# YJxyzxyz/road-vision-system

Hardware: AMD Instinct MI355X
Metric: end-to-end frames/sec @1080p (preproc+YOLOv8n+SORT), 1/2/4/8 MI355X (higher is better)
Workload: dtype bf16

## Files before the change

road-vision-system_amd/csrc/conv.hip:

```cpp
#include <algorithm>
#include <cstdlib>
#include <cstring>
#include "conv.h"
#include "conv_common.h"

namespace rv {

template <int MR, int NR, int WC>
__global__ __launch_bounds__(256, 2) void conv_mfma_kernel(ConvArgs a) {
  constexpr int WP = 4 / WC;
  const int tid = threadIdx.x;
  const int wave = tid >> 6, lane = tid & 63;
  const int col = lane & 15, quad = lane >> 4;
  const int wp = wave % WP, wc = wave / WP;
  const int cout_pad = (a.Cout + 15) & ~15;
  const int cout0 = (blockIdx.y * WC + wc) * (16 * MR);
  const int HWo = a.Ho * a.Wo;
  const int M = a.B * HWo;
  const int pix0 = (blockIdx.x * WP + wp) * (16 * NR);
  if (cout0 >= cout_pad || pix0 >= M) return;

  const int cin_pad = (a.Cin + 31) & ~31;
  const int kspt = cin_pad >> 5;
  const int Kp = a.k * a.k * cin_pad;
  const int nks = a.k * kspt;
  const int total = a.k * nks;

  const bf16_t* wrow[MR];
#pragma unroll
  for (int m = 0; m < MR; ++m) {
    int r = cout0 + m * 16 + col;
    r = r < cout_pad ? r : cout_pad - 1;
    wrow[m] = a.w + (size_t)r * Kp + quad * 8;
  }
  int iy0[NR], ix0[NR], pb[NR];
  bool pv[NR];
#pragma unroll
  for (int n = 0; n < NR; ++n) {
    const int p = pix0 + n * 16 + col;
    pv[n] = p < M;
    const int pp = pv[n] ? p : 0;
    const int b = pp / HWo;
    const int r = pp - b * HWo;
    const int oy = r / a.Wo;
    const int ox = r - oy * a.Wo;
    iy0[n] = oy * a.stride - a.pad;
    ix0[n] = ox * a.stride - a.pad;
    pb[n] = b * a.Hin * a.Win * a.in_cs + a.in_co + quad * 8;
  }

  f32x4 acc[MR][NR];
#pragma unroll
  for (int m = 0; m < MR; ++m)
#pragma unroll
    for (int n = 0; n < NR; ++n) acc[m][n] = f32x4{0.f, 0.f, 0.f, 0.f};

  const uint4 zero4 = make_uint4(0, 0, 0, 0);
  auto load = [&](int s, bf16x8 (&A)[MR], bf16x8 (&Bf)[NR]) {
    const int ky = s / nks;
    const int r = s - ky * nks;
    const int kx = r / kspt;
    const int cs = r - kx * kspt;
    const int kcol = s * 32;
#pragma unroll
    for (int m = 0; m < MR; ++m) A[m] = __builtin_bit_cast(bf16x8, *(const uint4*)(wrow[m] + kcol));
    const bool cvalid = cs * 32 + quad * 8 < a.Cin;
#pragma unroll
    for (int n = 0; n < NR; ++n) {
      const int iy = iy0[n] + ky, ix = ix0[n] + kx;
      const bool ok = pv[n] && cvalid && (unsigned)iy < (unsigned)a.Hin &&
                      (unsigned)ix < (unsigned)a.Win;
      uint4 v = zero4;
      if (ok)
        v = *(const uint4*)(a.in + (size_t)pb[n] + ((size_t)iy * a.Win + ix) * a.in_cs + cs * 32);
      Bf[n] = __builtin_bit_cast(bf16x8, v);
    }
  };
  auto mma = [&](const bf16x8 (&A)[MR], const bf16x8 (&Bf)[NR]) {
#pragma unroll
    for (int m = 0; m < MR; ++m)
#pragma unroll
      for (int n = 0; n < NR; ++n)
        acc[m][n] = __builtin_amdgcn_mfma_f32_16x16x32_bf16(A[m], Bf[n], acc[m][n], 0, 0, 0);
  };
  bf16x8 A0[MR], B0[NR], A1[MR], B1[NR];
  load(0, A0, B0);
  for (int s = 0; s < total; s += 2) {
    if (s + 1 < total) load(s + 1, A1, B1);
    mma(A0, B0);
    if (s + 1 >= total) break;
    if (s + 2 < total) load(s + 2, A0, B0);
    mma(A1, B1);
  }

#pragma unroll
  for (int n = 0; n < NR; ++n) {
    if (!pv[n]) continue;
    const int p = pix0 + n * 16 + col;
    const int b = p / HWo;
    const int r = p - b * HWo;
    const int oy = r / a.Wo;
    const int ox = r - oy * a.Wo;
    const size_t opix = (size_t)p;
#pragma unroll
    for (int m = 0; m < MR; ++m) {
      const int co = cout0 + m * 16 + quad * 4;
      if (co >= a.Cout) continue;
      float v[4];
      const float4 bb = *(const float4*)(a.bias + co);
      v[0] = acc[m][n][0] + bb.x;
      v[1] = acc[m][n][1] + bb.y;
      v[2] = acc[m][n][2] + bb.z;
      v[3] = acc[m][n][3] + bb.w;
      if (a.act) {
        silu4(v);
      }
      if (a.res) {
        const uint2 rr = *(const uint2*)(a.res + opix * a.res_cs + a.res_co + co);
        v[0] += bf2f(rr.x & 0xFFFF);
        v[1] += bf2f(rr.x >> 16);
        v[2] += bf2f(rr.y & 0xFFFF);
        v[3] += bf2f(rr.y >> 16);
      }
#pragma unroll
      for (int d = 0; d < 2; ++d) {
        void* outp = d == 0 ? a.out0 : a.out1;
        if (!outp) continue;
        const int cs_ = d == 0 ? a.out0_cs : a.out1_cs;
        const int co_ = (d == 0 ? a.out0_co : a.out1_co) + co;
        const int up = d == 0 ? a.out0_up : a.out1_up;
        if (a.out_f32) {
          float* o = (float*)outp;
          const float4 pk = make_float4(v[0], v[1], v[2], v[3]);
          if (!up) {
            *(float4*)(o + opix * cs_ + co_) = pk;
          } else {
            for (int dy = 0; dy < 2; ++dy)
              for (int dx = 0; dx < 2; ++dx) {
                const size_t q = ((size_t)(b * 2 * a.Ho + 2 * oy + dy) * (2 * a.Wo) + 2 * ox + dx);
                *(float4*)(o + q * cs_ + co_) = pk;
              }
          }
        } else {
          uint16_t* o = (uint16_t*)outp;
          const uint2 pk = make_uint2(pack_bf16x2(v[0], v[1]), pack_bf16x2(v[2], v[3]));
          if (!up) {
            *(uint2*)(o + opix * cs_ + co_) = pk;
          } else {
            for (int dy = 0; dy < 2; ++dy)
              for (int dx = 0; dx < 2; ++dx) {
                const size_t q = ((size_t)(b * 2 * a.Ho + 2 * oy + dy) * (2 * a.Wo) + 2 * ox + dx);
                *(uint2*)(o + q * cs_ + co_) = pk;
              }
          }
        }
      }
    }
  }
}

template <int MR, int NR, int WC>
static void launch_t(const ConvArgs& a, hipStream_t s) {
  constexpr int WP = 4 / WC;
  const int M = a.B * a.Ho * a.Wo;
  const int T = (a.Cout + 15) / 16;
  dim3 grid(ceil_div(M, 16 * NR * WP), ceil_div(T, MR * WC));
  conv_mfma_kernel<MR, NR, WC><<<grid, 256, 0, s>>>(a);
}

static int try_launch_patch(const ConvArgs& a, hipStream_t s, int* st);

static bool vcat(const ConvArgs& a) { return a.split > 0 || a.in_up; }

int launch_conv(const ConvArgs& a, hipStream_t s) {
  int st = 0;
  if (vcat(a)) {
    const int T = (a.Cout + 15) / 16;
    ConvCfg c{1, 1, 1, 1, 1, 1};
    for (const int mr : {8, 4, 2})
      if (T % mr == 0 && conv_cfg_ok(a, ConvCfg{mr, 1, 1, 1, 1, 1})) {
        c.mr = mr;
        break;
      }
    if (!conv_cfg_ok(a, c)) {
      set_error("virtual concat input (split %d, up %d) needs a bf16 1x1 conv", a.split, a.in_up);
      return RV_EINVAL;
    }
    return launch_conv_cfg(a, c, s);
  }
  if (try_launch_patch(a, s, &st)) return st;
  if (a.ch_w) {
    set_error("chained 1x1 conv (Cout %d, k%d s%d) has no patch-kernel configuration", a.Cout, a.k,
              a.stride);
    return RV_EINVAL;
  }
  if (a.in8) {
    set_error("fp8 conv (Cin %d, Cout %d, k%d s%d) has no patch-kernel configuration", a.Cin,
              a.Cout, a.k, a.stride);
    return RV_EINVAL;
  }
  if (a.g2_cout0 > 0) {
    set_error("grouped conv (Cout %d, split %d) has no patch-kernel configuration", a.Cout,
              a.g2_cout0);
    return RV_EINVAL;
  }
  const int T = (a.Cout + 15) / 16;
  const long M = (long)a.B * a.Ho * a.Wo;
  struct Cand {
    int mr, nr;
  };
  static const Cand cands[] = {{4, 4}, {2, 8}, {4, 2}, {2, 4}, {1, 8}, {4, 1}, {2, 2},
                               {1, 4}, {2, 1}, {1, 2}, {1, 1}};
  int MR = 1, NR = 1;
  for (const Cand& c : cands) {
    if (c.mr > T) continue;
    const int waste = ceil_div(T, c.mr) * c.mr - T;
    if (waste > 1 && c.mr > 1) continue;
    const long waves = (long)ceil_div((int)((M + 16 * c.nr - 1) / (16 * c.nr)), 1) * ceil_div(T, c.mr);
    MR = c.mr;
    NR = c.nr;
    if (waves >= 2048) break;
  }
  const int groups_c = ceil_div(T, MR);
  const int WC = groups_c >= 4 ? 4 : (groups_c >= 2 ? 2 : 1);
#define RV_CONV_WC(mr, nr)                                           \
  if (MR == mr && NR == nr) {                                        \
    if (WC == 4) launch_t<mr, nr, 4>(a, s);                          \
    else if (WC == 2) launch_t<mr, nr, 2>(a, s);                     \
    else launch_t<mr, nr, 1>(a, s);                                  \
    return launch_status("conv_mfma");                               \
  }
  RV_CONV_WC(4, 4) RV_CONV_WC(2, 8) RV_CONV_WC(4, 2) RV_CONV_WC(2, 4) RV_CONV_WC(1, 8)
  RV_CONV_WC(4, 1) RV_CONV_WC(2, 2) RV_CONV_WC(1, 4) RV_CONV_WC(2, 1) RV_CONV_WC(1, 2)
  RV_CONV_WC(1, 1)
#undef RV_CONV_WC
  set_error("no conv variant for MR=%d NR=%d", MR, NR);
  return RV_EINVAL;
}

__device__ __attribute__((aligned(64))) uint4 g_zero16[4];
#ifdef RV_PHASE_PROF
__device__ unsigned long long g_conv_phase[8];
#define RV_PH_T() __builtin_amdgcn_s_memtime()
#endif

struct TileWalk {
  int t0, step, end;
  __device__ __forceinline__ int count() const { return t0 < end ? (end - t0 + step - 1) / step : 0; }
};
__device__ __forceinline__ TileWalk tile_walk(int ntiles) {
  const int gx = gridDim.x, bx = blockIdx.x;
  if ((gx & 7) == 0) {
    const int chunk = (ntiles + 7) >> 3, j = bx & 7;
    return TileWalk{j * chunk + (bx >> 3), gx >> 3, min(ntiles, (j + 1) * chunk)};
  }
  return TileWalk{bx, gx, ntiles};
}
static inline int xcd_grid(int want, int ntiles, bool persist) {
  if (!persist) return ntiles >= 8 ? (ntiles + 7) & ~7 : ntiles;
  const int g = std::min(want, ntiles);
  return g >= 8 ? g & ~7 : g;
}

__device__ __forceinline__ void dma16(__amdgpu_buffer_rsrc_t r, void* lds, uint32_t voff, int soff) {
  __builtin_amdgcn_raw_ptr_buffer_load_lds(r, (__attribute__((address_space(3))) void*)lds, 16,
                                           (int)voff, soff, 0, 0);
}

struct PatchGeo {
  int C, R;
  int G;
  int PH, PW;
  int pinst;
  int tiles_x, tiles_y;
  int p_bytes;
  int fast;
};

static bool epi_fast(const ConvArgs& a) {
  const double px = (double)a.B * a.Ho * a.Wo;
  return !a.out_f32 && !a.out1 && !a.out0_up && !a.in8 && a.Cout % 16 == 0 && px < (1 << 23) &&
         a.out0_cs < 2048 && px * a.out0_cs * 2 < 2147483647.0 &&
         (!a.res || (a.res_cs < 2048 && px * a.res_cs * 2 < 2147483647.0));
}

template <int MR, int NR>
__device__ __forceinline__ void epilogue_fast(const ConvArgs& a, f32x4 (&acc)[MR][NR], int cout0,
                                              const bool (&pv)[NR], const uint32_t (&opx)[NR],
                                              int quad, const f32x4 (&bias)[MR]) {
  const __amdgpu_buffer_rsrc_t ro = __builtin_amdgcn_make_buffer_rsrc(a.out0, 0, 0x7FFFFFFF, kRsrcFlags);
  const __amdgpu_buffer_rsrc_t rr =
      __builtin_amdgcn_make_buffer_rsrc((void*)a.res, 0, 0x7FFFFFFF, kRsrcFlags);
  const int cq = cout0 + quad * 4;
  constexpr uint32_t kDrop = 0x80000000u;
  auto value = [&](int m, int n, uint32_t vr, uint32_t& lo, uint32_t& hi) {
    float v[4];
#pragma unroll
    for (int i = 0; i < 4; ++i) v[i] = acc[m][n][i] + bias[m][i];
    if (a.act) {
      silu4(v);
    }
    if (a.res) {
      const uint32_t roff = cout0 + m * 16 < a.Cout ? vr + m * 32 : kDrop;
      const uint2 q = __builtin_bit_cast(
          uint2, __builtin_amdgcn_raw_buffer_load_b64(rr, (int)roff, 0, 0));
      v[0] += bf2f(q.x & 0xFFFF);
      v[1] += bf2f(q.x >> 16);
      v[2] += bf2f(q.y & 0xFFFF);
      v[3] += bf2f(q.y >> 16);
    }
    lo = pack_bf16x2(v[0], v[1]);
    hi = pack_bf16x2(v[2], v[3]);
  };
#pragma unroll
  for (int n = 0; n < NR; ++n) {
    if (!pv[n]) continue;
    const uint32_t vo = (__umul24(opx[n], (uint32_t)a.out0_cs) + a.out0_co + cq) * 2;
    const uint32_t vr = a.res ? (__umul24(opx[n], (uint32_t)a.res_cs) + a.res_co + cq) * 2 : 0u;
    const uint32_t vo16 = vo + (16 * (quad & 1) + 8 * (quad >> 1) - 4 * quad) * 2;
#pragma unroll
    for (int m = 0; m + 1 < MR; m += 2) {
      if (cout0 + m * 16 >= a.Cout) continue;
      uint32_t a0, a1, b0, b1;
      value(m, n, vr, a0, a1);
      value(m + 1, n, vr, b0, b1);
      const auto x0 = __builtin_amdgcn_permlane16_swap(a0, b0, false, false);
      const auto x1 = __builtin_amdgcn_permlane16_swap(a1, b1, false, false);
      const bool ok = cout0 + (m + (quad & 1)) * 16 < a.Cout;
      const uint32_t off = ok ? vo16 + m * 32 : kDrop;
      const v4u32 pk = {x0[0], x1[0], x0[1], x1[1]};
      __builtin_amdgcn_raw_buffer_store_b128(pk, ro, (int)off, 0, 0);
    }
    if constexpr (MR & 1) {
      constexpr int m = MR - 1;
      if (cout0 + m * 16 < a.Cout) {
        uint32_t lo, hi;
        value(m, n, vr, lo, hi);
        __builtin_amdgcn_raw_buffer_store_b64(v2u32{lo, hi}, ro, (int)(vo + m * 32), 0, 0);
      }
    }
  }
}

template <int MR, int NR>
struct EpiPend {
  v4u32 pk[MR / 2 > 0 ? MR / 2 : 1][NR];
  uint32_t off[MR / 2 > 0 ? MR / 2 : 1][NR];
  v2u32 pk1[NR];
  uint32_t off1[NR];
};

template <int MR, int NR>
__device__ __forceinline__ void epi_pack(const ConvArgs& a, f32x4 (&acc)[MR][NR], int cout0,
                                         const bool (&pv)[NR], const uint32_t (&opx)[NR], int quad,
                                         const f32x4 (&bias)[MR], EpiPend<MR, NR>& ep) {
  const __amdgpu_buffer_rsrc_t rr =
      __builtin_amdgcn_make_buffer_rsrc((void*)a.res, 0, 0x7FFFFFFF, kRsrcFlags);
  const int cq = cout0 + quad * 4;
  constexpr uint32_t kDrop = 0x80000000u;
  uint2 rq[MR][NR];
  if (a.res) {
#pragma unroll
    for (int n = 0; n < NR; ++n) {
      const uint32_t vr = (__umul24(opx[n], (uint32_t)a.res_cs) + a.res_co + cq) * 2;
#pragma unroll
      for (int m = 0; m < MR; ++m) {
        const uint32_t roff = pv[n] && cout0 + m * 16 < a.Cout ? vr + m * 32 : kDrop;
        rq[m][n] = __builtin_bit_cast(uint2, __builtin_amdgcn_raw_buffer_load_b64(rr, (int)roff, 0, 0));
      }
    }
  }
  auto value = [&](int m, int n, uint32_t vr, uint32_t& lo, uint32_t& hi) {
    (void)vr;
    float v[4];
#pragma unroll
    for (int i = 0; i < 4; ++i) v[i] = acc[m][n][i] + bias[m][i];
    if (a.act) silu4(v);
    if (a.res) {
      const uint2 q = rq[m][n];
      v[0] += bf2f(q.x & 0xFFFF);
      v[1] += bf2f(q.x >> 16);
      v[2] += bf2f(q.y & 0xFFFF);
      v[3] += bf2f(q.y >> 16);
    }
    lo = pack_bf16x2(v[0], v[1]);
    hi = pack_bf16x2(v[2], v[3]);
  };
#pragma unroll
  for (int n = 0; n < NR; ++n) {
    const uint32_t vo = (__umul24(opx[n], (uint32_t)a.out0_cs) + a.out0_co + cq) * 2;
    const uint32_t vr = a.res ? (__umul24(opx[n], (uint32_t)a.res_cs) + a.res_co + cq) * 2 : 0u;
    const uint32_t vo16 = vo + (16 * (quad & 1) + 8 * (quad >> 1) - 4 * quad) * 2;
#pragma unroll
    for (int m = 0; m + 1 < MR; m += 2) {
      uint32_t a0, a1, b0, b1;
      value(m, n, vr, a0, a1);
      value(m + 1, n, vr, b0, b1);
      const auto x0 = __builtin_amdgcn_permlane16_swap(a0, b0, false, false);
      const auto x1 = __builtin_amdgcn_permlane16_swap(a1, b1, false, false);
      const bool ok = pv[n] && cout0 + (m + (quad & 1)) * 16 < a.Cout;
      ep.off[m / 2][n] = ok ? vo16 + m * 32 : kDrop;
      ep.pk[m / 2][n] = v4u32{x0[0], x1[0], x0[1], x1[1]};
    }
    if constexpr (MR & 1) {
      constexpr int m = MR - 1;
      uint32_t lo, hi;
      value(m, n, vr, lo, hi);
      ep.off1[n] = pv[n] && cout0 + m * 16 < a.Cout ? vo + m * 32 : kDrop;
      ep.pk1[n] = v2u32{lo, hi};
    }
  }
}

template <int MR, int NR>
__device__ __forceinline__ void epi_store(const ConvArgs& a, const EpiPend<MR, NR>& ep) {
  const __amdgpu_buffer_rsrc_t ro = __builtin_amdgcn_make_buffer_rsrc(a.out0, 0, 0x7FFFFFFF, kRsrcFlags);
#pragma unroll
  for (int n = 0; n < NR; ++n) {
#pragma unroll
    for (int m = 0; m + 1 < MR; m += 2)
      __builtin_amdgcn_raw_buffer_store_b128(ep.pk[m / 2][n], ro, (int)ep.off[m / 2][n], 0, 0);
    if constexpr (MR & 1) __builtin_amdgcn_raw_buffer_store_b64(ep.pk1[n], ro, (int)ep.off1[n], 0, 0);
  }
}

template <bool F8>
__device__ __forceinline__ int swzq(int i) {
  return F8 ? (i >> 2) & 3 : (i >> 1) & 2;
}

template <int MR, int NR>
__device__ __forceinline__ void epilogue(const ConvArgs& a, f32x4 (&acc)[MR][NR], int cout0,
                                         const bool (&pv)[NR], const int (&pb)[NR],
                                         const int (&py)[NR], const int (&px)[NR], int quad,
                                         const f32x4 (&bias)[MR]) {
#pragma unroll
  for (int n = 0; n < NR; ++n) {
    if (!pv[n]) continue;
    const int b = pb[n], oy = py[n], ox = px[n];
    const size_t opix = ((size_t)b * a.Ho + oy) * a.Wo + ox;
#pragma unroll
    for (int m = 0; m < MR; ++m) {
      const int co = cout0 + m * 16 + quad * 4;
      if (co >= a.Cout) continue;
      float v[4];
      v[0] = acc[m][n][0] + bias[m][0];
      v[1] = acc[m][n][1] + bias[m][1];
      v[2] = acc[m][n][2] + bias[m][2];
      v[3] = acc[m][n][3] + bias[m][3];
      if (a.act) {
        silu4(v);
      }
      if (a.res) {
        const uint2 rr = *(const uint2*)(a.res + opix * a.res_cs + a.res_co + co);
        v[0] += bf2f(rr.x & 0xFFFF);
        v[1] += bf2f(rr.x >> 16);
        v[2] += bf2f(rr.y & 0xFFFF);
        v[3] += bf2f(rr.y >> 16);
      }
#pragma unroll
      for (int d = 0; d < 2; ++d) {
        void* outp = d == 0 ? a.out0 : a.out1;
        if (!outp) continue;
        const int cs_ = d == 0 ? a.out0_cs : a.out1_cs;
        const int co_ = (d == 0 ? a.out0_co : a.out1_co) + co;
        const int up = d == 0 ? a.out0_up : a.out1_up;
        if (a.out_f32) {
          float* o = (float*)outp;
          const float4 pk = make_float4(v[0], v[1], v[2], v[3]);
          if (!up) {
            *(float4*)(o + opix * cs_ + co_) = pk;
          } else {
            for (int dy = 0; dy < 2; ++dy)
              for (int dx = 0; dx < 2; ++dx) {
                const size_t q = ((size_t)(b * 2 * a.Ho + 2 * oy + dy) * (2 * a.Wo) + 2 * ox + dx);
                *(float4*)(o + q * cs_ + co_) = pk;
              }
          }
        } else {
          uint16_t* o = (uint16_t*)outp;
          const uint2 pk = make_uint2(pack_bf16x2(v[0], v[1]), pack_bf16x2(v[2], v[3]));
          if (!up) {
            *(uint2*)(o + opix * cs_ + co_) = pk;
          } else {
            for (int dy = 0; dy < 2; ++dy)
              for (int dx = 0; dx < 2; ++dx) {
                const size_t q = ((size_t)(b * 2 * a.Ho + 2 * oy + dy) * (2 * a.Wo) + 2 * ox + dx);
                *(uint2*)(o + q * cs_ + co_) = pk;
              }
          }
        }
      }
    }
  }
}

template <int S>
constexpr int patch_pixb() {
  return 64;
}
template <int S>
__device__ __forceinline__ int patch_scol(int px, int PW) {
  return S == 1 ? px : ((px & 1) ? (PW + 1) / 2 + (px >> 1) : (px >> 1));
}

template <int NR, int S>
constexpr int patch_maxit() {
  return (S == 2 ? 6 : 2) * NR + 2;
}

template <int MR, int NR>
__device__ __forceinline__ void epilogue8(const ConvArgs& a, f32x4 (&acc)[MR][NR], int cout0,
                                          const bool (&pv)[NR], const int (&pb)[NR],
                                          const int (&py)[NR], const int (&px)[NR], int quad,
                                          const f32x4 (&bias)[MR], const f32x4 (&dq)[MR]) {
  const float inv0 = 1.0f / a.s_out0, inv1 = 1.0f / a.s_out1;
#pragma unroll
  for (int n = 0; n < NR; ++n) {
    if (!pv[n]) continue;
    const int b = pb[n], oy = py[n], ox = px[n];
    const size_t opix = ((size_t)b * a.Ho + oy) * a.Wo + ox;
#pragma unroll
    for (int m = 0; m < MR; ++m) {
      const int co = cout0 + m * 16 + quad * 4;
      if (co >= a.Cout) continue;
      float v[4];
#pragma unroll
      for (int i = 0; i < 4; ++i) v[i] = acc[m][n][i] * dq[m][i] + bias[m][i];
      if (a.act) {
        silu4(v);
      }
      if (a.res) {
        const uint32_t rr = *(const uint32_t*)((const uint8_t*)a.res + opix * a.res_cs + a.res_co + co);
        v[0] += __builtin_amdgcn_cvt_f32_fp8((int)rr, 0) * a.s_res;
        v[1] += __builtin_amdgcn_cvt_f32_fp8((int)rr, 1) * a.s_res;
        v[2] += __builtin_amdgcn_cvt_f32_fp8((int)rr, 2) * a.s_res;
        v[3] += __builtin_amdgcn_cvt_f32_fp8((int)rr, 3) * a.s_res;
      }
#pragma unroll
      for (int d = 0; d < 2; ++d) {
        void* outp = d == 0 ? a.out0 : a.out1;
        if (!outp) continue;
        const int cs_ = d == 0 ? a.out0_cs : a.out1_cs;
        const int co_ = (d == 0 ? a.out0_co : a.out1_co) + co;
        const int up = d == 0 ? a.out0_up : a.out1_up;
        const int o8 = d == 0 ? a.out0_8 : a.out1_8;
        const int ny = up ? 2 : 1;
        for (int dy = 0; dy < ny; ++dy)
          for (int dx = 0; dx < ny; ++dx) {
            const size_t q = up ? ((size_t)(b * 2 * a.Ho + 2 * oy + dy) * (2 * a.Wo) + 2 * ox + dx) : opix;
            if (o8) {
              *(uint32_t*)((uint8_t*)outp + q * cs_ + co_) = f8_encode4(v, d == 0 ? inv0 : inv1);
            } else if (a.out_f32) {
              *(float4*)((float*)outp + q * cs_ + co_) = make_float4(v[0], v[1], v[2], v[3]);
            } else {
              *(uint2*)((uint16_t*)outp + q * cs_ + co_) =
                  make_uint2(pack_bf16x2(v[0], v[1]), pack_bf16x2(v[2], v[3]));
            }
          }
      }
    }
  }
}

template <int MR, int NR, int K, int S, bool RESW, bool F8, int NW = 4, bool CH = false>
__global__ __launch_bounds__(64 * NW, NW == 4 ? 2 : 1) void conv_patch_kernel(ConvArgs a, PatchGeo g) {
  extern __shared__ __attribute__((aligned(16))) uint8_t smem[];
  constexpr int T2 = K * K;
  constexpr int BC = 16 * MR;
  constexpr int W_BYTES = BC * T2 * 64;
  constexpr int MAXP = patch_maxit<NR, S>();
  static_assert(MAXP <= 32, "tail mask is 32 bits");
  constexpr int WJ = BC * T2 / 16;
  constexpr int MAXW = (WJ + NW - 1) / NW;
  constexpr int EB = F8 ? 1 : 2;
  constexpr int CC = F8 ? 64 : 32;
  const int tid = threadIdx.x;
  const int wave = __builtin_amdgcn_readfirstlane(tid >> 6), lane = tid & 63;
  const int col = lane & 15, quad = lane >> 4;
  const int cout0 = blockIdx.y * BC;
  int wc0 = cout0, gcout = a.g2_cout0 > 0 ? a.g2_cout0 : a.Cout;
  int in_co = a.in_co, Cin = a.Cin;
  const uint8_t* wts = (const uint8_t*)a.w;
  const float* bias_p = a.bias;
  const float* wsc_p = a.wscale;
  if (a.g2_cout0 > 0 && cout0 >= a.g2_cout0) {
    wc0 = cout0 - a.g2_cout0;
    gcout = a.Cout - a.g2_cout0;
    in_co = a.g2_in_co;
    Cin = a.g2_Cin;
    wts = (const uint8_t*)a.g2_w;
    bias_p = a.g2_bias;
    wsc_p = a.g2_wscale;
  }
  const int wcout_pad = (gcout + 15) & ~15;
  const int cin_pad = (Cin + CC - 1) & ~(CC - 1);
  const int Kp = T2 * cin_pad;
  const int nch = cin_pad / CC;
  const int G = g.G < nch ? g.G : nch;
  const int ngrp = (nch + G - 1) / G;
  const int chunk_bytes = g.p_bytes + (RESW ? 0 : W_BYTES);
  const int stage_bytes = G * chunk_bytes;
  uint8_t* const stages = smem + (RESW ? nch * W_BYTES : 0);
  constexpr int pad = K / 2;
  const int tiles_img = g.tiles_x * g.tiles_y;
  const int ntiles = a.B * tiles_img;
  const TileWalk walk = tile_walk(ntiles);
  const int nsteps = walk.count() * ngrp;
  const int npp = g.PH * g.PW;
  const float inv_pw = 1.0f / (float)g.PW;

  constexpr int PB = patch_pixb<S>(), SL = PB / 16;
  int orow[NR], ocol[NR], boff[NR][K];
  bool oin[NR];
#pragma unroll
  for (int n = 0; n < NR; ++n) {
    const int q = wave * (NR * 16) + n * 16 + col;
    orow[n] = q / g.C;
    ocol[n] = q - orow[n] * g.C;
    oin[n] = q < g.R * g.C;
    const int pr = oin[n] ? orow[n] * S : 0, pc = oin[n] ? ocol[n] * S : 0;
#pragma unroll
    for (int kx = 0; kx < K; ++kx) {
      const int sc = patch_scol<S>(pc + kx, g.PW);
      const int lq = F8 ? quad >> 1 : quad;
      if constexpr (F8 && K == 3)
        boff[n][kx] = (pr * g.PW + sc) * 64 + swzq<true>(sc);
      else
        boff[n][kx] = (pr * g.PW + sc) * 64 + ((lq ^ swzq<F8>(sc)) << 4) + (F8 ? (quad & 1) * 8 : 0);
    }
  }
  int aoff[F8 && K == 3 ? MR : 1][2];
  if constexpr (F8 && K == 3) {
#pragma unroll
    for (int m = 0; m < MR; ++m) {
      const int row = m * 16 + col, sw = swzq<true>(row);
      const int base = (row * T2 + (quad >> 1)) * 64;
      aoff[m][0] = base + (((2 * (quad & 1)) ^ sw) << 4);
      aoff[m][1] = base + (((2 * (quad & 1) + 1) ^ sw) << 4);
    }
  }
  float* const bias_lds = (float*)(stages + 2 * stage_bytes);
  f32x4 bias[F8 ? MR : 1], dq[F8 ? MR : 1];
  if constexpr (F8) {
#pragma unroll
    for (int m = 0; m < MR; ++m) {
      const int co = wc0 + m * 16 + quad * 4;
      bias[m] = co < wcout_pad ? *(const f32x4*)(bias_p + co) : f32x4{0.f, 0.f, 0.f, 0.f};
      const f32x4 ws = co < wcout_pad ? *(const f32x4*)(wsc_p + co) : f32x4{0.f, 0.f, 0.f, 0.f};
      dq[m] = ws * a.s_in;
    }
  } else {
    for (int i = tid; i < BC; i += 64 * NW) bias_lds[i] = wc0 + i < wcout_pad ? bias_p[wc0 + i] : 0.f;
  }
  auto bias_tile = [&](f32x4 (&bl)[MR]) {
#pragma unroll
    for (int m = 0; m < MR; ++m) bl[m] = *(const f32x4*)(bias_lds + m * 16 + quad * 4);
  };
  constexpr int CHN = (MR + 1) / 2;
  uint8_t* const ch_w_lds = (uint8_t*)(bias_lds + BC);
  float* const ch_b_lds = (float*)(ch_w_lds + (CH ? CHN * BC * 64 : 0));
  uint8_t* const ch_x_lds = (uint8_t*)(ch_b_lds + (CH ? BC : 0)) + wave * (CH ? CHN * NR * 16 * 64 : 0);
  if constexpr (CH) {
    static_assert(!F8 && K == 3 && MR % 2 == 0, "chained 1x1: bf16 behind a 3x3 conv, fragment pairs");
    for (int j = wave; j < CHN * (BC / 16); j += NW) {
      const int c = j / (BC / 16), jr = j - c * (BC / 16);
      const int row = jr * 16 + (lane >> 2);
      const int q = (lane & 3) ^ swzq<false>(row);
      __builtin_amdgcn_global_load_lds((const void*)(a.ch_w + (size_t)row * (CHN * 32) + c * 32 + q * 8),
                                       (void*)(ch_w_lds + c * BC * 64 + jr * 1024), 16, 0, 0);
    }
    for (int i = tid; i < BC; i += 64 * NW) ch_b_lds[i] = a.ch_b[i];
  }
  uint32_t tailbad = 0;
  int lgeo[MAXP];
#pragma unroll
  for (int it = 0; it < MAXP; ++it) {
    const int L = 64 * (wave + NW * it) + lane;
    const int pix = L / SL, q = L - SL * pix;
    const int py = (int)(((float)pix + 0.5f) * inv_pw);
    const int sc = pix - py * g.PW;
    const int he = (g.PW + 1) >> 1;
    const int px = S == 1 ? sc : (sc < he ? 2 * sc : 2 * (sc - he) + 1);
    const int sq = q ^ swzq<F8>(sc);
    lgeo[it] = (pix < npp ? py : 4095) | (px << 12) | (sq << 24);
    if ((nch - 1) * CC + sq * (16 / EB) >= Cin) tailbad |= 1u << it;
  }
  const bool has_tail = Cin % CC != 0;
  uint32_t voff[MAXP];
  __amdgpu_buffer_rsrc_t img_rsrc;
  const int pix_bytes = a.in_cs * EB;
  auto prep_tile = [&](int ti) {
    const int b = ti / tiles_img;
    const int r = ti - b * tiles_img;
    const int ty = r / g.tiles_x, tx = r - (r / g.tiles_x) * g.tiles_x;
    const int iy0 = ty * g.R * S - pad, ix0 = tx * g.C * S - pad;
    const uint8_t* base = (const uint8_t*)a.in + ((size_t)b * a.Hin * a.Win * a.in_cs + in_co) * EB;
    img_rsrc = __builtin_amdgcn_make_buffer_rsrc((void*)base, 0,
                                                 (a.Hin * a.Win * a.in_cs - in_co) * EB, kRsrcFlags);
#pragma unroll
    for (int it = 0; it < MAXP; ++it) {
      const int gg = lgeo[it];
      const int iy = iy0 + (gg & 4095), ix = ix0 + ((gg >> 12) & 4095);
      const bool ok = (unsigned)iy < (unsigned)a.Hin && (unsigned)ix < (unsigned)a.Win;
      const uint32_t off = __umul24((uint32_t)(__umul24(iy, a.Win) + ix), (uint32_t)pix_bytes) +
                           ((gg >> 24) & 3) * 16;
      const uint32_t m = ok ? 0u : 0xFFFFFFFFu;
      voff[it] = (off & ~m) | (kOOB & m);
    }
  };
  const __amdgpu_buffer_rsrc_t w_rsrc = __builtin_amdgcn_make_buffer_rsrc(
      (void*)(wts + (size_t)wc0 * Kp * EB), 0, (wcout_pad - wc0) * Kp * EB, kRsrcFlags);
  uint32_t wvoff[MAXW];
#pragma unroll
  for (int it = 0; it < MAXW; ++it) {
    const int j = wave + NW * it;
    const int pr = j * 16 + (lane >> 2);
    const int row = pr / T2, tap = pr - (pr / T2) * T2;
    const int q = (lane & 3) ^ swzq<F8>(row);
    wvoff[it] = wc0 + row < wcout_pad ? (uint32_t)((row * Kp + tap * cin_pad) * EB + q * 16) : kOOB;
  }
  auto dma_weights = [&](int c, uint8_t* Wl) {
#pragma unroll
    for (int it = 0; it < MAXW; ++it) {
      const int j = wave + NW * it;
      if (j < WJ) dma16(w_rsrc, Wl + j * 1024, wvoff[it], c * 64);
    }
  };
  auto stage = [&](int grp, int buf) {
    for (int gi = 0; gi < G; ++gi) {
      const int c = grp * G + gi;
      if (c >= nch) break;
      uint8_t* P = stages + buf * stage_bytes + gi * chunk_bytes;
      const bool tail = has_tail && c == nch - 1;
      if (tail) {
#pragma unroll
        for (int it = 0; it < MAXP; ++it) {
          const int j = wave + NW * it;
          if (j < g.pinst)
            dma16(img_rsrc, P + j * 1024, tail && ((tailbad >> it) & 1) ? kOOB : voff[it], c * 64);
        }
      } else {
#pragma unroll
        for (int it = 0; it < MAXP; ++it) {
          const int j = wave + NW * it;
          if (j < g.pinst) dma16(img_rsrc, P + j * 1024, voff[it], c * 64);
        }
      }
      if constexpr (!RESW) dma_weights(c, P + g.p_bytes);
    }
  };
  f32x4 acc[MR][NR];
  auto compute = [&](int grp, int buf) {
    for (int gi = 0; gi < G; ++gi) {
      const int c = grp * G + gi;
      if (c >= nch) break;
      const uint8_t* P = stages + buf * stage_bytes + gi * chunk_bytes;
      const uint8_t* Wl = RESW ? smem + c * W_BYTES : P + g.p_bytes;
      if constexpr (F8 && K == 3) {
        const int rowb = g.PW * PB;
#pragma unroll
        for (int t = 0; t < 9; t += 2) {
          const bool odd = t + 1 >= 9;
          const int ky0 = t / 3, kx0 = t % 3;
          const int ky1 = odd ? ky0 : (t + 1) / 3, kx1 = odd ? kx0 : (t + 1) % 3;
          const bool hi = (quad >> 1) != 0;
          i32x8 A[MR], Bv[NR];
#pragma unroll
          for (int m = 0; m < MR; ++m) {
            const uint4 lo = *(const uint4*)(Wl + aoff[m][0] + t * 64);
            const uint4 up = *(const uint4*)(Wl + aoff[m][1] + t * 64);
            A[m] = i32x8{(int)lo.x, (int)lo.y, (int)lo.z, (int)lo.w,
                         (int)up.x, (int)up.y, (int)up.z, (int)up.w};
            if (odd && hi) A[m] = i32x8{0, 0, 0, 0, 0, 0, 0, 0};
          }
#pragma unroll
          for (int n = 0; n < NR; ++n) {
            const int v = hi ? boff[n][kx1] + ky1 * rowb : boff[n][kx0] + ky0 * rowb;
            const int sw = v & 3, base = v & ~63;
            const uint4 lo = *(const uint4*)(P + base + (((2 * (quad & 1)) ^ sw) << 4));
            const uint4 up = *(const uint4*)(P + base + (((2 * (quad & 1) + 1) ^ sw) << 4));
            Bv[n] = i32x8{(int)lo.x, (int)lo.y, (int)lo.z, (int)lo.w,
                          (int)up.x, (int)up.y, (int)up.z, (int)up.w};
          }
#pragma unroll
          for (int m = 0; m < MR; ++m)
#pragma unroll
            for (int n = 0; n < NR; ++n)
              acc[m][n] = __builtin_amdgcn_mfma_scale_f32_16x16x128_f8f6f4(
                  A[m], Bv[n], acc[m][n], 0, 0, 0, 127, 0, 127);
        }
        continue;
      }
      if constexpr (!F8 && MR * NR < 16) {
        bf16x8 Af[2][MR], Bq[2][NR];
        auto ld = [&](int tap, int sl) {
          const int ky = tap / K, kx = tap - (tap / K) * K;
#pragma unroll
          for (int m = 0; m < MR; ++m) {
            const int row = m * 16 + col;
            Af[sl][m] = __builtin_bit_cast(
                bf16x8, *(const uint4*)(Wl + (row * T2 + tap) * 64 + ((quad ^ swzq<false>(row)) << 4)));
          }
#pragma unroll
          for (int n = 0; n < NR; ++n)
            Bq[sl][n] = __builtin_bit_cast(bf16x8, *(const uint4*)(P + ky * g.PW * PB + boff[n][kx]));
        };
        ld(0, 0);
#pragma unroll
        for (int t = 0; t < T2; ++t) {
          if (t + 1 < T2) ld(t + 1, (t + 1) & 1);
          __builtin_amdgcn_sched_barrier(0);
#pragma unroll
          for (int m = 0; m < MR; ++m)
#pragma unroll
            for (int n = 0; n < NR; ++n)
              acc[m][n] = __builtin_amdgcn_mfma_f32_16x16x32_bf16(Af[t & 1][m], Bq[t & 1][n],
                                                                  acc[m][n], 0, 0, 0);
          __builtin_amdgcn_sched_barrier(0);
        }
        continue;
      }
#pragma unroll(F8 || MR * NR >= 16 ? 1 : K)
      for (int ky = 0; ky < K; ++ky) {
        const uint8_t* Prow = P + ky * g.PW * PB;
#pragma unroll
        for (int kx = 0; kx < K; ++kx) {
          const int tap = ky * K + kx;
          if constexpr (F8) {
#pragma unroll
            for (int hh = 0; hh < 2; ++hh) {
              long A[MR], Bf[NR];
#pragma unroll
              for (int m = 0; m < MR; ++m) {
                const int row = m * 16 + col;
                A[m] = *(const long*)(Wl + (((row * T2 + tap) * 64 +
                                             (((quad >> 1) ^ swzq<true>(row)) << 4) + (quad & 1) * 8) ^
                                            (hh << 5)));
              }
#pragma unroll
              for (int n = 0; n < NR; ++n) Bf[n] = *(const long*)(Prow + (boff[n][kx] ^ (hh << 5)));
              __builtin_amdgcn_sched_barrier(0);
#pragma unroll
              for (int m = 0; m < MR; ++m)
#pragma unroll
                for (int n = 0; n < NR; ++n)
                  acc[m][n] = __builtin_amdgcn_mfma_f32_16x16x32_fp8_fp8(A[m], Bf[n], acc[m][n], 0, 0, 0);
            }
          } else {
            bf16x8 A[MR], Bf[NR];
#pragma unroll
            for (int m = 0; m < MR; ++m) {
              const int row = m * 16 + col;
              A[m] = __builtin_bit_cast(
                  bf16x8, *(const uint4*)(Wl + (row * T2 + tap) * 64 + ((quad ^ swzq<false>(row)) << 4)));
            }
#pragma unroll
            for (int n = 0; n < NR; ++n)
              Bf[n] = __builtin_bit_cast(bf16x8, *(const uint4*)(Prow + boff[n][kx]));
            __builtin_amdgcn_sched_barrier(0);
#pragma unroll
            for (int m = 0; m < MR; ++m)
#pragma unroll
              for (int n = 0; n < NR; ++n)
                acc[m][n] = __builtin_amdgcn_mfma_f32_16x16x32_bf16(A[m], Bf[n], acc[m][n], 0, 0, 0);
          }
        }
      }
    }
  };

  if (nsteps == 0) return;
#ifdef RV_PHASE_PROF
  unsigned long long ph[5] = {0, 0, 0, 0, 0}, t_ph = RV_PH_T();
#define RV_PH(i)                             \
  {                                          \
    const unsigned long long t_ = RV_PH_T(); \
    ph[i] += t_ - t_ph;                      \
    t_ph = t_;                               \
  }
#else
#define RV_PH(i)
#endif
  int ti = walk.t0;
  int grp = 0;
  constexpr bool kDefer = !F8 && !CH && MR * NR <= 10;
  auto chain_tile = [&](const bool (&pv)[NR], const uint32_t (&opx)[NR]) {
    if constexpr (CH) {
      f32x4 bl[MR];
      bias_tile(bl);
#pragma unroll
      for (int n = 0; n < NR; ++n) {
        const int px = n * 16 + col;
#pragma unroll
        for (int m = 0; m < MR; m += 2) {
          uint32_t v0[2], v1[2];
#pragma unroll
          for (int h = 0; h < 2; ++h) {
            float v[4];
#pragma unroll
            for (int i = 0; i < 4; ++i) v[i] = acc[m + h][n][i] + bl[m + h][i];
            if (a.act) silu4(v);
            v0[h] = pack_bf16x2(v[0], v[1]);
            v1[h] = pack_bf16x2(v[2], v[3]);
          }
          const auto x0 = __builtin_amdgcn_permlane16_swap(v0[0], v0[1], false, false);
          const auto x1 = __builtin_amdgcn_permlane16_swap(v1[0], v1[1], false, false);
          const int qq = 2 * (quad & 1) + (quad >> 1);
          *(v4u32*)(ch_x_lds + ((m / 2) * NR * 16 + px) * 64 + ((qq ^ swzq<false>(px)) << 4)) =
              v4u32{x0[0], x1[0], x0[1], x1[1]};
        }
      }
      f32x4 acc2[MR][NR];
#pragma unroll
      for (int m = 0; m < MR; ++m)
#pragma unroll
        for (int n = 0; n < NR; ++n) acc2[m][n] = f32x4{0.f, 0.f, 0.f, 0.f};
#pragma unroll
      for (int c = 0; c < CHN; ++c) {
        bf16x8 A2[MR], B2[NR];
#pragma unroll
        for (int m = 0; m < MR; ++m) {
          const int row = m * 16 + col;
          A2[m] = __builtin_bit_cast(
              bf16x8, *(const uint4*)(ch_w_lds + c * BC * 64 + row * 64 + ((quad ^ swzq<false>(row)) << 4)));
        }
#pragma unroll
        for (int n = 0; n < NR; ++n) {
          const int px = n * 16 + col;
          B2[n] = __builtin_bit_cast(
              bf16x8, *(const uint4*)(ch_x_lds + (c * NR * 16 + px) * 64 + ((quad ^ swzq<false>(px)) << 4)));
        }
#pragma unroll
        for (int m = 0; m < MR; ++m)
#pragma unroll
          for (int n = 0; n < NR; ++n)
            acc2[m][n] = __builtin_amdgcn_mfma_f32_16x16x32_bf16(A2[m], B2[n], acc2[m][n], 0, 0, 0);
      }
      f32x4 bl2[MR];
#pragma unroll
      for (int m = 0; m < MR; ++m) bl2[m] = *(const f32x4*)(ch_b_lds + m * 16 + quad * 4);
      ConvArgs a2 = a;
      a2.act = 1;
      a2.res = nullptr;
      epilogue_fast<MR, NR>(a2, acc2, 0, pv, opx, quad, bl2);
    }
  };
  auto finish = [&](int tile, EpiPend<MR, NR>& ep) {
    const int b = tile / tiles_img;
    const int r = tile - b * tiles_img;
    const int ty = r / g.tiles_x, tx = r - (r / g.tiles_x) * g.tiles_x;
    bool pv[NR];
    int pb[NR], py[NR], px[NR];
#pragma unroll
    for (int n = 0; n < NR; ++n) {
      pb[n] = b;
      py[n] = ty * g.R + orow[n];
      px[n] = tx * g.C + ocol[n];
      pv[n] = oin[n] && py[n] < a.Ho && px[n] < a.Wo;
    }
    if constexpr (F8) {
      epilogue8<MR, NR>(a, acc, cout0, pv, pb, py, px, quad, bias, dq);
    } else if constexpr (CH) {
      uint32_t opx[NR];
#pragma unroll
      for (int n = 0; n < NR; ++n) opx[n] = (uint32_t)((b * a.Ho + py[n]) * a.Wo + px[n]);
      chain_tile(pv, opx);
    } else if (g.fast) {
      uint32_t opx[NR];
#pragma unroll
      for (int n = 0; n < NR; ++n) opx[n] = __umul24((uint32_t)(b * a.Ho + py[n]), (uint32_t)a.Wo) + px[n];
      f32x4 bl[MR];
      bias_tile(bl);
      if constexpr (kDefer)
        epi_pack<MR, NR>(a, acc, cout0, pv, opx, quad, bl, ep);
      else
        epilogue_fast<MR, NR>(a, acc, cout0, pv, opx, quad, bl);
    } else {
      f32x4 bl[MR];
      bias_tile(bl);
      epilogue<MR, NR>(a, acc, cout0, pv, pb, py, px, quad, bl);
    }
  };
  if constexpr (RESW)
    for (int c = 0; c < nch; ++c) dma_weights(c, smem + c * W_BYTES);
  prep_tile(ti);
  stage(0, 0);
  __syncthreads();
  RV_PH(0);
  for (int s = 0; s < nsteps; ++s) {
    EpiPend<MR, NR> ep;
    if (grp == 0) {
#pragma unroll
      for (int m = 0; m < MR; ++m)
#pragma unroll
        for (int n = 0; n < NR; ++n) acc[m][n] = f32x4{0.f, 0.f, 0.f, 0.f};
    }
    const bool last = grp + 1 == ngrp;
    if (s + 1 < nsteps) {
      if (last) prep_tile(ti + walk.step);
      stage(last ? 0 : grp + 1, (s + 1) & 1);
    }
    RV_PH(1);
    compute(grp, s & 1);
    RV_PH(2);
    if (last) {
      finish(ti, ep);
      ti += walk.step;
      grp = 0;
      RV_PH(3);
    } else {
      ++grp;
    }
    __syncthreads();
    if constexpr (kDefer) {
      if (last && g.fast) epi_store<MR, NR>(a, ep);
    }
    RV_PH(4);
  }
#ifdef RV_PHASE_PROF
  if (lane == 0) {
#pragma unroll
    for (int i = 0; i < 5; ++i) atomicAdd(&g_conv_phase[i], ph[i]);
    atomicAdd(&g_conv_phase[5], (unsigned long long)nsteps);
    atomicAdd(&g_conv_phase[6], 1ull);
  }
#endif
#undef RV_PH
}


template <int MR, int NR>
__global__ __launch_bounds__(256, 2) void conv1x1_direct_kernel(ConvArgs a, int fast) {
  extern __shared__ __attribute__((aligned(16))) uint8_t smem[];
  constexpr int BC = 16 * MR;
  constexpr int W_BYTES = BC * 64;
  constexpr int WJ = BC / 16;
  constexpr int MAXW = (WJ + 3) / 4;
  const int tid = threadIdx.x;
  const int wave = tid >> 6, lane = tid & 63;
  const int col = lane & 15, quad = lane >> 4;
  const int cout0 = blockIdx.y * BC;
  const int wcout_pad = (a.Cout + 15) & ~15;
  const int cin_pad = (a.Cin + 31) & ~31;
  const int nch = cin_pad >> 5;
  const int HW = a.Ho * a.Wo;
  const int npix = a.B * HW;
  const int ntiles = (npix + 64 * NR - 1) / (64 * NR);
  for (int c = 0; c < nch; ++c) {
#pragma unroll
    for (int it = 0; it < MAXW; ++it) {
      const int j = wave + 4 * it;
      if (j < WJ) {
        const int row = j * 16 + (lane >> 2);
        const int q = (lane & 3) ^ swzq<false>(row);
        const int co = cout0 + row;
        const void* src = co < wcout_pad ? (const void*)(a.w + (size_t)co * cin_pad + q * 8 + c * 32)
                                         : (const void*)g_zero16;
        __builtin_amdgcn_global_load_lds(src, (void*)(smem + c * W_BYTES + j * 1024), 16, 0, 0);
      }
    }
  }
  __syncthreads();
  f32x4 bias[MR];
#pragma unroll
  for (int m = 0; m < MR; ++m) {
    const int co = cout0 + m * 16 + quad * 4;
    bias[m] = co < wcout_pad ? *(const f32x4*)(a.bias + co) : f32x4{0.f, 0.f, 0.f, 0.f};
  }
  int aoff[MR];
#pragma unroll
  for (int m = 0; m < MR; ++m) {
    const int row = m * 16 + col;
    aoff[m] = row * 64 + ((quad ^ swzq<false>(row)) << 4);
  }
  const bool need_geo = a.in_up || !fast;
  const TileWalk walk = tile_walk(ntiles);
  struct Geo {
    const bf16_t* src[NR];
    const bf16_t* src2[NR];
    bool pv[NR];
    int pb[NR], py[NR], px[NR];
  };
  auto geo = [&](int t, Geo& G) {
#pragma unroll
    for (int n = 0; n < NR; ++n) {
      const int p = t * 64 * NR + wave * 16 * NR + n * 16 + col;
      G.pv[n] = t < walk.end && p < npix;
      const int pp = G.pv[n] ? p : 0;
      G.pb[n] = G.py[n] = G.px[n] = 0;
      if (need_geo) {
        G.pb[n] = pp / HW;
        const int r = pp - G.pb[n] * HW;
        G.py[n] = r / a.Wo;
        G.px[n] = r - G.py[n] * a.Wo;
      }
      const size_t ps = a.in_up ? ((size_t)G.pb[n] * (a.Ho >> 1) + (G.py[n] >> 1)) * (a.Wo >> 1) +
                                      (G.px[n] >> 1)
                                : (size_t)pp;
      G.src[n] = a.in + ps * a.in_cs + a.in_co + quad * 8;
      G.src2[n] = a.in2 + (size_t)pp * a.in2_cs + a.in2_co + quad * 8 - a.split;
    }
  };
  auto load = [&](const Geo& G, int c, uint4 (&B)[NR]) {
    const bool kin = c * 32 + quad * 8 < a.Cin;
    const bool second = a.split > 0 && c * 32 >= a.split;
#pragma unroll
    for (int n = 0; n < NR; ++n)
      B[n] = *(const uint4*)((G.pv[n] && kin) ? (const void*)((second ? G.src2[n] : G.src[n]) + c * 32)
                                              : (const void*)g_zero16);
  };
  auto mma = [&](int c, const uint4 (&B)[NR], f32x4 (&acc)[MR][NR]) {
    const uint8_t* Wl = smem + c * W_BYTES;
    bf16x8 A[MR];
#pragma unroll
    for (int m = 0; m < MR; ++m) A[m] = __builtin_bit_cast(bf16x8, *(const uint4*)(Wl + aoff[m]));
    __builtin_amdgcn_sched_barrier(0);
#pragma unroll
    for (int m = 0; m < MR; ++m)
#pragma unroll
      for (int n = 0; n < NR; ++n)
        acc[m][n] = __builtin_amdgcn_mfma_f32_16x16x32_bf16(A[m], __builtin_bit_cast(bf16x8, B[n]),
                                                            acc[m][n], 0, 0, 0);
  };
  auto finish = [&](int t, const Geo& G, f32x4 (&acc)[MR][NR]) {
    if (fast) {
      uint32_t opx[NR];
#pragma unroll
      for (int n = 0; n < NR; ++n) opx[n] = (uint32_t)(t * 64 * NR + wave * 16 * NR + n * 16 + col);
      epilogue_fast<MR, NR>(a, acc, cout0, G.pv, opx, quad, bias);
    } else {
      epilogue<MR, NR>(a, acc, cout0, G.pv, G.pb, G.py, G.px, quad, bias);
    }
  };
  const int P = (nch + 1) & ~1;
  uint4 B0[NR], B1[NR];
  Geo G0, G1;
  int t = walk.t0;
  geo(t, G0);
  geo(t + walk.step, G1);
  load(G0, 0, B0);
  load(G0, 1, B1);
  for (; t < walk.end; t += walk.step) {
    f32x4 acc[MR][NR];
#pragma unroll
    for (int m = 0; m < MR; ++m)
#pragma unroll
      for (int n = 0; n < NR; ++n) acc[m][n] = f32x4{0.f, 0.f, 0.f, 0.f};
    for (int c = 0; c < P - 2; c += 2) {
      mma(c, B0, acc);
      __builtin_amdgcn_sched_barrier(0);
      load(G0, c + 2, B0);
      __builtin_amdgcn_sched_barrier(0);
      mma(c + 1, B1, acc);
      __builtin_amdgcn_sched_barrier(0);
      load(G0, c + 3, B1);
      __builtin_amdgcn_sched_barrier(0);
    }
    mma(P - 2, B0, acc);
    __builtin_amdgcn_sched_barrier(0);
    load(G1, 0, B0);
    __builtin_amdgcn_sched_barrier(0);
    if (P - 1 < nch) mma(P - 1, B1, acc);
    __builtin_amdgcn_sched_barrier(0);
    load(G1, 1, B1);
    __builtin_amdgcn_sched_barrier(0);
    finish(t, G0, acc);
    G0 = G1;
    geo(t + 2 * walk.step, G1);
  }
}

static int conv_nch(const ConvArgs& a) {
  int cin = a.Cin;
  if (a.g2_cout0 > 0 && a.g2_Cin > cin) cin = a.g2_Cin;
  const int cc = a.in8 ? 64 : 32;
  return (cin + cc - 1) / cc;
}

static bool patch_geo(const ConvArgs& a, const ConvCfg& c, PatchGeo& g, size_t& smem) {
  if (!((a.k == 1 || a.k == 3) && (a.stride == 1 || a.stride == 2) && a.pad == a.k / 2)) return false;
  if ((size_t)a.Hin * a.Win >= (1u << 24) || (size_t)a.in_cs * 2 >= (1u << 24)) return false;
  const int NR = c.nr, MR = c.mr;
  const int NW = c.kind == 2 ? 8 : 4;
  const int P = 16 * NR * NW;
  struct TileKey {
    int wo, ho, s, k, p, c;
  };
  static thread_local TileKey memo[64];
  static thread_local int memo_n = 0, memo_w = 0;
  int C = 0;
  for (int i = 0; i < memo_n && !C; ++i)
    if (memo[i].wo == a.Wo && memo[i].ho == a.Ho && memo[i].s == a.stride && memo[i].k == a.k &&
        memo[i].p == P)
      C = memo[i].c;
  if (!C) {
    long best = -1;
    for (int c = std::min(a.Wo, P); c >= std::min(16, a.Wo); --c) {
      const int r = P / c;
      const long cost = (long)ceil_div(a.Wo, c) * ceil_div(a.Ho, r) * ((r - 1) * a.stride + a.k) *
                        ((c - 1) * a.stride + a.k);
      if (best < 0 || cost < best) {
        best = cost;
        C = c;
      }
    }
    memo[memo_w++ & 63] = TileKey{a.Wo, a.Ho, a.stride, a.k, P, C};
    memo_n = std::min(memo_n + 1, 64);
  }
  g.C = C;
  g.R = P / C;
  if (g.R < 1) return false;
  g.PH = (g.R - 1) * a.stride + a.k;
  g.PW = (g.C - 1) * a.stride + a.k;
  g.pinst = ceil_div(g.PH * g.PW * 4, 64);
  g.p_bytes = g.pinst * 1024;
  g.tiles_x = ceil_div(a.Wo, g.C);
  g.tiles_y = ceil_div(a.Ho, g.R);
  const int nch = conv_nch(a);
  g.G = std::max(1, std::min(c.G, nch));
  g.fast = epi_fast(a) ? 1 : 0;
  const int maxit = (a.stride == 2 ? 6 : 2) * NR + 2;
  if (ceil_div(g.pinst, NW) > maxit) return false;
  const size_t wb = (size_t)16 * MR * a.k * a.k * 64;
  smem = (c.resw ? nch * wb : 0) + 2 * (size_t)g.G * (g.p_bytes + (c.resw ? 0 : wb)) +
         (a.in8 ? 0 : (size_t)16 * MR * 4);
  if (a.ch_w) {
    const size_t chn = (MR + 1) / 2;
    smem += chn * 16 * MR * 64 + (size_t)16 * MR * 4 + (size_t)NW * chn * NR * 16 * 64;
  }
  return smem <= 160 * 1024;
}

template <int MR, int NR, int K, int S, bool RESW, bool F8 = false, int NW = 4, bool CH = false>
static int launch_patch_t(const ConvArgs& a, const PatchGeo& g, size_t smem, int persist,
                          hipStream_t s) {
  static bool attr = false;
  auto fn = conv_patch_kernel<MR, NR, K, S, RESW, F8, NW, CH>;
  if (!attr) {
    hipError_t e = hipFuncSetAttribute((const void*)fn, hipFuncAttributeMaxDynamicSharedMemorySize,
                                       160 * 1024);
    if (e != hipSuccess) {
      (void)hipGetLastError();
      set_error("hipFuncSetAttribute: %s", hipGetErrorString(e));
      return -(int)e;
    }
    attr = true;
  }
  static size_t occ_smem[16] = {0};
  static int occ_val[16] = {0};
  int occ = 0;
  for (int i = 0; i < 16; ++i)
    if (occ_smem[i] == smem) occ = occ_val[i];
  if (!occ) {
    if (hipOccupancyMaxActiveBlocksPerMultiprocessor(&occ, fn, 64 * NW, smem) != hipSuccess || occ < 1)
      occ = 1;
    (void)hipGetLastError();
    for (int i = 0; i < 16; ++i)
      if (occ_smem[i] == 0) {
        occ_smem[i] = smem;
        occ_val[i] = occ;
        break;
      }
  }
  const int T = (a.Cout + 15) / 16;
  const int ytiles = ceil_div(T, MR);
  const int ntiles = a.B * g.tiles_x * g.tiles_y;
  const int gx = xcd_grid(std::max(1, num_cus() * occ / ytiles), ntiles, persist != 0);
  dim3 grid(gx, ytiles);
  fn<<<grid, 64 * NW, smem, s>>>(a, g);
  return launch_status("conv_patch");
}

static size_t direct_smem(const ConvArgs& a, int MR) {
  return (size_t)((a.Cin + 31) / 32) * 16 * MR * 64;
}

template <int MR, int NR>
static int launch_direct_t(const ConvArgs& a, int persist, hipStream_t s) {
  static bool attr = false;
  auto fn = conv1x1_direct_kernel<MR, NR>;
  if (!attr) {
    hipError_t e = hipFuncSetAttribute((const void*)fn, hipFuncAttributeMaxDynamicSharedMemorySize,
                                       160 * 1024);
    if (e != hipSuccess) {
      (void)hipGetLastError();
      set_error("hipFuncSetAttribute: %s", hipGetErrorString(e));
      return -(int)e;
    }
    attr = true;
  }
  const size_t smem = direct_smem(a, MR);
  static size_t occ_smem[16] = {0};
  static int occ_val[16] = {0};
  int occ = 0;
  for (int i = 0; i < 16; ++i)
    if (occ_smem[i] == smem) occ = occ_val[i];
  if (!occ) {
    if (hipOccupancyMaxActiveBlocksPerMultiprocessor(&occ, fn, 256, smem) != hipSuccess || occ < 1)
      occ = 1;
    (void)hipGetLastError();
    for (int i = 0; i < 16; ++i)
      if (occ_smem[i] == 0) {
        occ_smem[i] = smem;
        occ_val[i] = occ;
        break;
      }
  }
  const int ytiles = ceil_div((a.Cout + 15) / 16, MR);
  const int ntiles = ceil_div(a.B * a.Ho * a.Wo, 64 * NR);
  const int gx = xcd_grid(std::max(1, num_cus() * occ / ytiles), ntiles, persist != 0);
  fn<<<dim3(gx, ytiles), 256, smem, s>>>(a, epi_fast(a) ? 1 : 0);
  return launch_status("conv1x1_direct");
}

static bool direct_ok(const ConvArgs& a, const ConvCfg& c) {
  const int T = (a.Cout + 15) / 16;
  const bool vcat_ok = (a.split == 0 && !a.in_up) ||
                       (a.split % 32 == 0 && a.split <= a.Cin && (!a.in_up || (a.Ho % 2 == 0 && a.Wo % 2 == 0)) &&
                        (a.split == a.Cin || (a.in2 && a.in2_cs % 8 == 0 && a.in2_co % 8 == 0)));
  return a.k == 1 && a.stride == 1 && a.pad == 0 && a.g2_cout0 <= 0 && a.Hin == a.Ho &&
         a.Win == a.Wo && (c.mr <= T || c.mr == 1) && a.in_cs % 8 == 0 && a.in_co % 8 == 0 &&
         !a.in8 && vcat_ok && direct_smem(a, c.mr) <= 160 * 1024;
}


template <int MR, int NR>
constexpr bool patch_s2_ok() {
  return NR <= 2 && MR * NR <= 8;
}

constexpr bool patch_spills(int MR, int NR, int K, int S, bool RESW) {
  return !RESW && K == 3 && ((S == 1 && MR * NR > 16) || (S == 2 && MR * NR >= 8));
}

template <int MR, int NR>
constexpr bool tile8_built() {
  return (MR == 1 || MR == 2 || MR == 4) && (NR == 1 || NR == 2 || NR == 4);
}
constexpr bool patch_spills8(int MR, int NR, int K, int S, bool RESW) {
  return K == 3 && (MR * NR >= 16 || (S == 1 && MR == 2 && NR == 4) ||
                    (S == 2 && !RESW && MR == 1 && NR == 2));
}

template <int MR, int NR>
constexpr bool ch_built() {
  return NR <= 2 && MR == 4;
}
static bool ch_tile_ok(int mr, int nr) { return nr <= 2 && mr == 4; }
template <int MR, int NR, bool RESW, int NW>
static int launch_patch_ch(const ConvArgs& a, const PatchGeo& g, size_t smem, int persist,
                           hipStream_t s) {
  if constexpr (ch_built<MR, NR>()) {
    if (a.k == 3 && a.stride == 2)
      return launch_patch_t<MR, NR, 3, 2, RESW, false, NW, true>(a, g, smem, persist, s);
    if (a.k == 3 && a.stride == 1)
      return launch_patch_t<MR, NR, 3, 1, RESW, false, NW, true>(a, g, smem, persist, s);
  }
  set_error("conv_patch (chained 1x1): no variant MR=%d NR=%d k=%d s=%d", MR, NR, a.k, a.stride);
  return RV_EINVAL;
}

template <int MR, int NR, bool RESW>
static int launch_patch_ks(const ConvArgs& a, const PatchGeo& g, size_t smem, int persist,
                           hipStream_t s) {
  if (a.ch_w) return launch_patch_ch<MR, NR, RESW, 4>(a, g, smem, persist, s);
  if (a.in8) {
    if constexpr (tile8_built<MR, NR>()) {
      if constexpr (!patch_spills(MR, NR, 3, 1, RESW) && !patch_spills8(MR, NR, 3, 1, RESW))
        if (a.k == 3 && a.stride == 1)
          return launch_patch_t<MR, NR, 3, 1, RESW, true>(a, g, smem, persist, s);
      if (a.k == 1 && a.stride == 1)
        return launch_patch_t<MR, NR, 1, 1, RESW, true>(a, g, smem, persist, s);
      if constexpr (patch_s2_ok<MR, NR>() && !patch_spills(MR, NR, 3, 2, RESW) &&
                    !patch_spills8(MR, NR, 3, 2, RESW)) {
        if (a.k == 3 && a.stride == 2)
          return launch_patch_t<MR, NR, 3, 2, RESW, true>(a, g, smem, persist, s);
      }
    }
    set_error("conv_patch (fp8): no variant MR=%d NR=%d k=%d s=%d", MR, NR, a.k, a.stride);
    return RV_EINVAL;
  }
  if constexpr (!patch_spills(MR, NR, 3, 1, RESW))
    if (a.k == 3 && a.stride == 1) return launch_patch_t<MR, NR, 3, 1, RESW>(a, g, smem, persist, s);
  if (a.k == 1 && a.stride == 1) return launch_patch_t<MR, NR, 1, 1, RESW>(a, g, smem, persist, s);
  if constexpr (patch_s2_ok<MR, NR>() && !patch_spills(MR, NR, 3, 2, RESW)) {
    if (a.k == 3 && a.stride == 2) return launch_patch_t<MR, NR, 3, 2, RESW>(a, g, smem, persist, s);
  }
  set_error("conv_patch: no variant MR=%d NR=%d k=%d s=%d", MR, NR, a.k, a.stride);
  return RV_EINVAL;
}

template <int MR, int NR>
constexpr bool tile_w8_built() {
  return (MR == 8 && NR <= 2) || (MR == 5 && NR <= 2) || (MR == 4 && NR <= 4 && NR != 3) ||
         (MR == 2 && (NR == 2 || NR == 4));
}
template <int MR, int NR, bool RESW>
static int launch_patch8_ks(const ConvArgs& a, const PatchGeo& g, size_t smem, int persist,
                            hipStream_t s) {
  if (a.ch_w) return launch_patch_ch<MR, NR, RESW, 8>(a, g, smem, persist, s);
  if constexpr (tile_w8_built<MR, NR>()) {
    if (!a.in8 && a.k == 3 && a.stride == 1)
      return launch_patch_t<MR, NR, 3, 1, RESW, false, 8>(a, g, smem, persist, s);
    if constexpr (patch_s2_ok<MR, NR>())
      if (!a.in8 && a.k == 3 && a.stride == 2)
        return launch_patch_t<MR, NR, 3, 2, RESW, false, 8>(a, g, smem, persist, s);
  }
  set_error("conv_patch (8 waves): no variant MR=%d NR=%d k=%d s=%d", MR, NR, a.k, a.stride);
  return RV_EINVAL;
}
static bool w8_tile(int mr, int nr) {
  return (mr == 8 && nr <= 2) || (mr == 5 && nr <= 2) || (mr == 4 && (nr == 1 || nr == 2 || nr == 4)) ||
         (mr == 2 && (nr == 2 || nr == 4));
}

static const int kTiles[][2] = {{8, 2}, {8, 1}, {5, 2}, {5, 1}, {4, 4}, {4, 2}, {4, 1},
                                {2, 4}, {2, 2}, {2, 1}, {1, 4}, {1, 2}, {1, 1}};

bool conv_cfg_ok(const ConvArgs& a, const ConvCfg& c) {
  if (a.ch_w &&
      (c.kind == 1 || a.in8 || !ch_tile_ok(c.mr, c.nr) || 16 * c.mr < a.Cout ||
       16 * c.mr - a.Cout >= 16 || a.k != 3 || a.res || a.out1 || a.out0_up || a.g2_cout0 > 0 ||
       vcat(a) || !epi_fast(a)))
    return false;
  if (c.kind == 1) return !a.in8 && direct_ok(a, c);
  if ((c.kind != 0 && c.kind != 2) || vcat(a)) return false;
  if (c.kind == 2 && (a.in8 || a.k != 3 || !w8_tile(c.mr, c.nr))) return false;
  if (a.in8 && !((c.mr == 1 || c.mr == 2 || c.mr == 4) && (c.nr == 1 || c.nr == 2 || c.nr == 4)))
    return false;
  if (a.in8 && (a.Cin % 16 || a.in_co % 16 || a.in_cs % 16 ||
                 (a.g2_cout0 > 0 && (a.g2_Cin % 16 || a.g2_in_co % 16))))
    return false;
  const int T = (a.Cout + 15) / 16;
  if (c.mr > T && c.mr > 1) return false;
  if (a.stride == 2 && (c.nr > 2 || c.mr * c.nr > 8 || a.k != 3)) return false;
  if (a.g2_cout0 > 0 && a.g2_cout0 % (16 * c.mr) != 0) return false;
  if (c.kind == 0 && patch_spills(c.mr, c.nr, a.k, a.stride, c.resw != 0)) return false;
  if (a.in8 && patch_spills8(c.mr, c.nr, a.k, a.stride, c.resw != 0)) return false;
  PatchGeo g;
  size_t sm;
  return patch_geo(a, c, g, sm);
}

#ifdef RV_PHASE_PROF
}
extern "C" int rv_conv_phase_read(unsigned long long* out, int reset) {
  if (hipMemcpyFromSymbol(out, HIP_SYMBOL(rv::g_conv_phase), 8 * sizeof(unsigned long long)) != hipSuccess)
    return -1;
  if (reset) {
    static const unsigned long long z[8] = {0, 0, 0, 0, 0, 0, 0, 0};
    if (hipMemcpyToSymbol(HIP_SYMBOL(rv::g_conv_phase), z, sizeof(z)) != hipSuccess) return -1;
  }
  return 0;
}
namespace rv {
#endif
int launch_conv_cfg(const ConvArgs& a, const ConvCfg& c, hipStream_t s) {
  PatchGeo g;
  size_t sm;
  if (!conv_cfg_ok(a, c) || (c.kind != 1 && !patch_geo(a, c, g, sm))) {
    set_error("conv config MR=%d NR=%d G=%d resw=%d not valid for this layer", c.mr, c.nr, c.G,
              c.resw);
    return RV_EINVAL;
  }
#define RV_PATCH(M_, N_)                                                                     \
  if (c.mr == M_ && c.nr == N_)                                                              \
    return c.kind == 1 ? launch_direct_t<M_, N_>(a, c.persist, s)                            \
           : c.kind == 2 ? (c.resw ? launch_patch8_ks<M_, N_, true>(a, g, sm, c.persist, s)    \
                                   : launch_patch8_ks<M_, N_, false>(a, g, sm, c.persist, s))  \
           : c.resw    ? launch_patch_ks<M_, N_, true>(a, g, sm, c.persist, s)               \
                       : launch_patch_ks<M_, N_, false>(a, g, sm, c.persist, s);
  RV_PATCH(8, 2) RV_PATCH(8, 1) RV_PATCH(5, 2) RV_PATCH(5, 1) RV_PATCH(4, 4) RV_PATCH(4, 2)
  RV_PATCH(4, 1) RV_PATCH(2, 4) RV_PATCH(2, 2) RV_PATCH(2, 1) RV_PATCH(1, 4) RV_PATCH(1, 2)
  RV_PATCH(1, 1)
#undef RV_PATCH
  set_error("no conv_patch tile MR=%d NR=%d", c.mr, c.nr);
  return RV_EINVAL;
}

int conv_candidates(const ConvArgs& a, ConvCfg* out, int cap) {
  int n = 0;
  const int nch = conv_nch(a);
  for (const auto& t : kTiles) {
    for (int kind = 0; kind <= 2; kind += 2)
      for (int resw = 1; resw >= 0; --resw) {
        int gbest = 0;
        for (int G = nch; G >= 1 && !gbest; --G)
          if (conv_cfg_ok(a, ConvCfg{t[0], t[1], G, resw, 1, kind})) gbest = G;
        if (!gbest) continue;
        for (int persist = 1; persist >= 0; --persist) {
          if (n < cap) out[n] = ConvCfg{t[0], t[1], gbest, resw, persist, kind};
          ++n;
          if (!resw && gbest > 1) {
            if (n < cap) out[n] = ConvCfg{t[0], t[1], 1, resw, persist, kind};
            ++n;
          }
        }
      }
    for (int persist = 1; persist >= 0; --persist) {
      const ConvCfg d{t[0], t[1], 1, 1, persist, 1};
      if (!a.in8 && direct_ok(a, d)) {
        if (n < cap) out[n] = d;
        ++n;
      }
    }
  }
  return n;
}

static bool default_cfg(const ConvArgs& a, ConvCfg& best) {
  const int T = (a.Cout + 15) / 16;
  double best_fill = -1.0;
  bool found = false;
  for (const auto& t : kTiles) {
    if (ceil_div(T, t[0]) * t[0] - T > (t[0] > 1 ? 1 : 0)) continue;
    if (a.k == 3 && t[0] > 5) continue;
    ConvCfg cand{0, 0, 0, 0, 1};
    bool ok = false;
    for (int resw = 1; resw >= 0 && !ok; --resw)
      for (int G = conv_nch(a); G >= 1 && !ok; --G) {
        cand = ConvCfg{t[0], t[1], G, resw, 1};
        ok = conv_cfg_ok(a, cand);
      }
    if (!ok) continue;
    PatchGeo g;
    size_t sm = 0;
    patch_geo(a, cand, g, sm);
    const long blocks = (long)a.B * g.tiles_x * g.tiles_y * ceil_div(T, t[0]);
    const int bpc = std::max(1, std::min(4, (int)((160 * 1024) / sm)));
    const double fill = (double)blocks / (256.0 * bpc);
    if (fill >= 0.75) {
      best = cand;
      return true;
    }
    if (fill > best_fill) {
      best_fill = fill;
      best = cand;
      found = true;
    }
  }
  return found;
}

static int try_launch_patch(const ConvArgs& a, hipStream_t s, int* st) {
  ConvCfg c{0, 0, 1, 0, 1};
  if (!default_cfg(a, c)) return 0;
  static const int dbg = getenv("RV_CONV_DEBUG") ? atoi(getenv("RV_CONV_DEBUG")) : 0;
  if (dbg)
    fprintf(stderr, "[conv] %dx%d k%d s%d Cin %d Cout %d -> MR=%d NR=%d G=%d resw=%d\n", a.Ho, a.Wo,
            a.k, a.stride, a.Cin, a.Cout, c.mr, c.nr, c.G, c.resw);
  *st = launch_conv_cfg(a, c, s);
  return 1;
}

}
extern "C" int rv_conv_bf16(const void* in, int B, int Hin, int Win, int Cin, int in_cs,
                            const void* w, const float* bias, int Cout, int k, int stride, void* out,
                            int out_cs, const void* res, int res_cs, int act, const int* cfg6,
                            void* stream) {
  using namespace rv;
  RV_CHECK_ARG(in && w && bias && out, "null pointer");
  RV_CHECK_ARG(B >= 1 && Hin >= 1 && Win >= 1 && Cin >= 1 && Cout >= 1, "bad shape");
  RV_CHECK_ARG((k == 1 || k == 3) && (stride == 1 || stride == 2), "k %d stride %d", k, stride);
  RV_CHECK_ARG(in_cs >= Cin && out_cs >= Cout && (!res || res_cs >= Cout), "channel strides");
  ConvArgs a;
  memset(&a, 0, sizeof(a));
  a.in = (const bf16_t*)in;
  a.in_cs = in_cs;
  a.Hin = Hin;
  a.Win = Win;
  a.Cin = Cin;
  a.w = (const bf16_t*)w;
  a.bias = bias;
  a.Cout = Cout;
  a.k = k;
  a.stride = stride;
  a.pad = k / 2;
  a.Ho = (Hin + 2 * a.pad - k) / stride + 1;
  a.Wo = (Win + 2 * a.pad - k) / stride + 1;
  a.B = B;
  a.out0 = out;
  a.out0_cs = out_cs;
  a.res = (const bf16_t*)res;
  a.res_cs = res_cs;
  a.act = act ? 1 : 0;
  const hipStream_t s = (hipStream_t)stream;
  if (cfg6) {
    const ConvCfg c{cfg6[0], cfg6[1], cfg6[2], cfg6[3], cfg6[4], cfg6[5]};
    return launch_conv_cfg(a, c, s);
  }
  return launch_conv(a, s);
}
```

road-vision-system_amd/csrc/conv_common.h:

```cpp
#pragma once
#include "conv.h"

namespace rv {

typedef __attribute__((ext_vector_type(8))) __bf16 bf16x8;
typedef __attribute__((ext_vector_type(4))) float f32x4;
typedef __attribute__((ext_vector_type(8))) int i32x8;

typedef __attribute__((ext_vector_type(2))) float f32x2v;
typedef __attribute__((ext_vector_type(2))) __bf16 bf16x2v;
typedef __attribute__((ext_vector_type(2))) unsigned int v2u32;
typedef __attribute__((ext_vector_type(4))) unsigned int v4u32;

__device__ __forceinline__ uint16_t f2bf(float f) { return __builtin_bit_cast(uint16_t, (__bf16)f); }
__device__ __forceinline__ uint32_t pack_bf16x2(float lo, float hi) {
  return __builtin_bit_cast(uint32_t, __builtin_convertvector(f32x2v{lo, hi}, bf16x2v));
}
__device__ __forceinline__ float bf2f(uint16_t h) { return __uint_as_float((uint32_t)h << 16); }

__device__ __forceinline__ float silu(float v) {
  return v * __builtin_amdgcn_rcpf(1.0f + __expf(-v));
}
__device__ __forceinline__ f32x2v silu2(f32x2v x) {
  const float nl2e = __builtin_bit_cast(float, 0xBFB8AA3Bu);
  const f32x2v t = x * f32x2v{nl2e, nl2e};
  const f32x2v d = f32x2v{__builtin_amdgcn_exp2f(t.x), __builtin_amdgcn_exp2f(t.y)} + 1.0f;
  return x * f32x2v{__builtin_amdgcn_rcpf(d.x), __builtin_amdgcn_rcpf(d.y)};
}
__device__ __forceinline__ void silu4(float (&v)[4]) {
  const f32x2v a = silu2(f32x2v{v[0], v[1]}), b = silu2(f32x2v{v[2], v[3]});
  v[0] = a.x;
  v[1] = a.y;
  v[2] = b.x;
  v[3] = b.y;
}

constexpr int kRsrcFlags = 0x00020000;
constexpr uint32_t kOOB = 0x80000000u;
__device__ __forceinline__ uint32_t f8_encode4(const float (&v)[4], float inv_s) {
  float q[4];
#pragma unroll
  for (int i = 0; i < 4; ++i) q[i] = fminf(fmaxf(v[i] * inv_s, -448.f), 448.f);
  int w = __builtin_amdgcn_cvt_pk_fp8_f32(q[0], q[1], 0, false);
  w = __builtin_amdgcn_cvt_pk_fp8_f32(q[2], q[3], w, true);
  return (uint32_t)w;
}

inline int num_cus() {
  static int n = 0;
  if (!n) {
    int dev = 0;
    hipDeviceProp_t p;
    if (hipGetDevice(&dev) == hipSuccess && hipGetDeviceProperties(&p, dev) == hipSuccess)
      n = p.multiProcessorCount;
    else
      n = 256;
    (void)hipGetLastError();
  }
  return n;
}

}
```

Baseline: 44170.

## Specialize conv epilogues on act/res, batch SiLU, use buffer loads and incremental tile walk

Templates the epilogue and pack paths on compile-time activation and residual flags, and batches SiLU evaluation across several rows so transcendental ops can be interleaved. The patch kernel now precomputes per-slot relative offsets and boundary bitmasks, visiting only live slots through a switch-based unroll. Tile coordinates advance incrementally instead of using a division per tile. The 1x1 direct kernel switches from raw pointer loads with a zero buffer to buffer-resource loads with out-of-bounds masking, and the generic epilogue reloads its arguments from the kernarg segment to lower register pressure. These changes target scalar/VGPR overhead and branches in hot loops. In exchange they add template instantiations, code size and new 32-bit range guards.

Result: no change. 44640, median of 2 (+1.1%).

```diff
diff --git a/road-vision-system_amd/csrc/conv.hip b/road-vision-system_amd/csrc/conv.hip
--- a/road-vision-system_amd/csrc/conv.hip
+++ b/road-vision-system_amd/csrc/conv.hip
@@ -1,6 +1,7 @@
 #include <algorithm>
 #include <cstdlib>
 #include <cstring>
+#include <type_traits>
 #include "conv.h"
 #include "conv_common.h"
 
@@ -267,6 +268,23 @@
                                            (int)voff, soff, 0, 0);
 }
 
+template <int MAXP, class F>
+__device__ __forceinline__ void for_live(int n, F&& f) {
+  static_assert(MAXP <= 16, "for_live: 16 slots");
+#define RV_SLOT(i)                                              \
+  case i + 1:                                                   \
+    if constexpr (i < MAXP) f(std::integral_constant<int, i>{}); \
+    [[fallthrough]];
+  switch (n) {
+    default:
+      RV_SLOT(15) RV_SLOT(14) RV_SLOT(13) RV_SLOT(12) RV_SLOT(11) RV_SLOT(10) RV_SLOT(9) RV_SLOT(8)
+      RV_SLOT(7) RV_SLOT(6) RV_SLOT(5) RV_SLOT(4) RV_SLOT(3) RV_SLOT(2) RV_SLOT(1) RV_SLOT(0)
+    case 0:
+      break;
+  }
+#undef RV_SLOT
+}
+
 struct PatchGeo {
   int C, R;
   int G;
@@ -284,61 +302,96 @@
          (!a.res || (a.res_cs < 2048 && px * a.res_cs * 2 < 2147483647.0));
 }
 
-template <int MR, int NR>
-__device__ __forceinline__ void epilogue_fast(const ConvArgs& a, f32x4 (&acc)[MR][NR], int cout0,
-                                              const bool (&pv)[NR], const uint32_t (&opx)[NR],
-                                              int quad, const f32x4 (&bias)[MR]) {
+template <int MR, bool ACT, bool RES>
+__device__ __forceinline__ void epi_col(float (&v)[MR][4], const uint2 (&rq)[MR], uint32_t vo,
+                                        bool pvn, int cout0, int Cout, int quad,
+                                        v4u32 (&pk)[MR / 2 > 0 ? MR / 2 : 1],
+                                        uint32_t (&off)[MR / 2 > 0 ? MR / 2 : 1], v2u32& pk1,
+                                        uint32_t& off1) {
+  constexpr uint32_t kDrop = 0x80000000u;
+  if constexpr (ACT) {
+    static_assert(MR <= 8, "two batches");
+    silu4_batch<(MR < 4 ? MR : 4)>(v);
+    if constexpr (MR > 4) silu4_batch<MR - 4>(v + 4);
+  }
+  if constexpr (RES) {
+#pragma unroll
+    for (int m = 0; m < MR; ++m) {
+      v[m][0] += bf2f(rq[m].x & 0xFFFF);
+      v[m][1] += bf2f(rq[m].x >> 16);
+      v[m][2] += bf2f(rq[m].y & 0xFFFF);
+      v[m][3] += bf2f(rq[m].y >> 16);
+    }
+  }
+  uint32_t lo[MR], hi[MR];
+#pragma unroll
+  for (int m = 0; m < MR; ++m) {
+    lo[m] = pack_bf16x2(v[m][0], v[m][1]);
+    hi[m] = pack_bf16x2(v[m][2], v[m][3]);
+  }
+  const uint32_t vo16 = vo + (16 * (quad & 1) + 8 * (quad >> 1) - 4 * quad) * 2;
+#pragma unroll
+  for (int m = 0; m + 1 < MR; m += 2) {
+    const auto x0 = __builtin_amdgcn_permlane16_swap(lo[m], lo[m + 1], false, false);
+    const auto x1 = __builtin_amdgcn_permlane16_swap(hi[m], hi[m + 1], false, false);
+    const bool ok = pvn && cout0 + (m + (quad & 1)) * 16 < Cout;
+    off[m / 2] = ok ? vo16 + m * 32 : kDrop;
+    pk[m / 2] = v4u32{x0[0], x1[0], x0[1], x1[1]};
+  }
+  if constexpr (MR & 1) {
+    constexpr int m = MR - 1;
+    off1 = pvn && cout0 + m * 16 < Cout ? vo + m * 32 : kDrop;
+    pk1 = v2u32{lo[m], hi[m]};
+  }
+}
+
+template <int MR, int NR, bool ACT, bool RES>
+__device__ __forceinline__ void epilogue_fast_t(const ConvArgs& a, f32x4 (&acc)[MR][NR], int cout0,
+                                                const bool (&pv)[NR], const uint32_t (&opx)[NR],
+                                                int quad, const f32x4 (&bias)[MR]) {
   const __amdgpu_buffer_rsrc_t ro = __builtin_amdgcn_make_buffer_rsrc(a.out0, 0, 0x7FFFFFFF, kRsrcFlags);
   const __amdgpu_buffer_rsrc_t rr =
       __builtin_amdgcn_make_buffer_rsrc((void*)a.res, 0, 0x7FFFFFFF, kRsrcFlags);
   const int cq = cout0 + quad * 4;
   constexpr uint32_t kDrop = 0x80000000u;
-  auto value = [&](int m, int n, uint32_t vr, uint32_t& lo, uint32_t& hi) {
-    float v[4];
-#pragma unroll
-    for (int i = 0; i < 4; ++i) v[i] = acc[m][n][i] + bias[m][i];
-    if (a.act) {
-      silu4(v);
-    }
-    if (a.res) {
-      const uint32_t roff = cout0 + m * 16 < a.Cout ? vr + m * 32 : kDrop;
-      const uint2 q = __builtin_bit_cast(
-          uint2, __builtin_amdgcn_raw_buffer_load_b64(rr, (int)roff, 0, 0));
-      v[0] += bf2f(q.x & 0xFFFF);
-      v[1] += bf2f(q.x >> 16);
-      v[2] += bf2f(q.y & 0xFFFF);
-      v[3] += bf2f(q.y >> 16);
-    }
-    lo = pack_bf16x2(v[0], v[1]);
-    hi = pack_bf16x2(v[2], v[3]);
-  };
 #pragma unroll
   for (int n = 0; n < NR; ++n) {
-    if (!pv[n]) continue;
+    uint2 rq[MR];
+    if constexpr (RES) {
+      const uint32_t vr = (__umul24(opx[n], (uint32_t)a.res_cs) + a.res_co + cq) * 2;
+#pragma unroll
+      for (int m = 0; m < MR; ++m) {
+        const uint32_t roff = pv[n] && cout0 + m * 16 < a.Cout ? vr + m * 32 : kDrop;
+        rq[m] = __builtin_bit_cast(uint2, __builtin_amdgcn_raw_buffer_load_b64(rr, (int)roff, 0, 0));
+      }
+    }
+    float v[MR][4];
+#pragma unroll
+    for (int m = 0; m < MR; ++m)
+#pragma unroll
+      for (int i = 0; i < 4; ++i) v[m][i] = acc[m][n][i] + bias[m][i];
     const uint32_t vo = (__umul24(opx[n], (uint32_t)a.out0_cs) + a.out0_co + cq) * 2;
-    const uint32_t vr = a.res ? (__umul24(opx[n], (uint32_t)a.res_cs) + a.res_co + cq) * 2 : 0u;
-    const uint32_t vo16 = vo + (16 * (quad & 1) + 8 * (quad >> 1) - 4 * quad) * 2;
-#pragma unroll
-    for (int m = 0; m + 1 < MR; m += 2) {
-      if (cout0 + m * 16 >= a.Cout) continue;
-      uint32_t a0, a1, b0, b1;
-      value(m, n, vr, a0, a1);
-      value(m + 1, n, vr, b0, b1);
-      const auto x0 = __builtin_amdgcn_permlane16_swap(a0, b0, false, false);
-      const auto x1 = __builtin_amdgcn_permlane16_swap(a1, b1, false, false);
-      const bool ok = cout0 + (m + (quad & 1)) * 16 < a.Cout;
-      const uint32_t off = ok ? vo16 + m * 32 : kDrop;
-      const v4u32 pk = {x0[0], x1[0], x0[1], x1[1]};
-      __builtin_amdgcn_raw_buffer_store_b128(pk, ro, (int)off, 0, 0);
-    }
-    if constexpr (MR & 1) {
-      constexpr int m = MR - 1;
-      if (cout0 + m * 16 < a.Cout) {
-        uint32_t lo, hi;
-        value(m, n, vr, lo, hi);
-        __builtin_amdgcn_raw_buffer_store_b64(v2u32{lo, hi}, ro, (int)(vo + m * 32), 0, 0);
-      }
-    }
+    v4u32 pk[MR / 2 > 0 ? MR / 2 : 1];
+    uint32_t off[MR / 2 > 0 ? MR / 2 : 1], off1;
+    v2u32 pk1;
+    epi_col<MR, ACT, RES>(v, rq, vo, pv[n], cout0, a.Cout, quad, pk, off, pk1, off1);
+#pragma unroll
+    for (int m = 0; m + 1 < MR; m += 2)
+      __builtin_amdgcn_raw_buffer_store_b128(pk[m / 2], ro, (int)off[m / 2], 0, 0);
+    if constexpr (MR & 1) __builtin_amdgcn_raw_buffer_store_b64(pk1, ro, (int)off1, 0, 0);
+  }
+}
+
+template <int MR, int NR>
+__device__ __forceinline__ void epilogue_fast(const ConvArgs& a, f32x4 (&acc)[MR][NR], int cout0,
+                                              const bool (&pv)[NR], const uint32_t (&opx)[NR],
+                                              int quad, const f32x4 (&bias)[MR]) {
+  if (a.act) {
+    if (a.res) epilogue_fast_t<MR, NR, true, true>(a, acc, cout0, pv, opx, quad, bias);
+    else epilogue_fast_t<MR, NR, true, false>(a, acc, cout0, pv, opx, quad, bias);
+  } else {
+    if (a.res) epilogue_fast_t<MR, NR, false, true>(a, acc, cout0, pv, opx, quad, bias);
+    else epilogue_fast_t<MR, NR, false, false>(a, acc, cout0, pv, opx, quad, bias);
   }
 }
 
@@ -350,65 +403,55 @@
   uint32_t off1[NR];
 };
 
+template <int MR, int NR, bool ACT, bool RES>
+__device__ __forceinline__ void epi_pack_t(const ConvArgs& a, f32x4 (&acc)[MR][NR], int cout0,
+                                           const bool (&pv)[NR], const uint32_t (&opx)[NR], int quad,
+                                           const f32x4 (&bias)[MR], EpiPend<MR, NR>& ep) {
+  const __amdgpu_buffer_rsrc_t rr =
+      __builtin_amdgcn_make_buffer_rsrc((void*)a.res, 0, 0x7FFFFFFF, kRsrcFlags);
+  const int cq = cout0 + quad * 4;
+  constexpr uint32_t kDrop = 0x80000000u;
+  uint2 rq[NR][MR];
+  if constexpr (RES) {
+#pragma unroll
+    for (int n = 0; n < NR; ++n) {
+      const uint32_t vr = (__umul24(opx[n], (uint32_t)a.res_cs) + a.res_co + cq) * 2;
+#pragma unroll
+      for (int m = 0; m < MR; ++m) {
+        const uint32_t roff = pv[n] && cout0 + m * 16 < a.Cout ? vr + m * 32 : kDrop;
+        rq[n][m] = __builtin_bit_cast(uint2, __builtin_amdgcn_raw_buffer_load_b64(rr, (int)roff, 0, 0));
+      }
+    }
+  }
+#pragma unroll
+  for (int n = 0; n < NR; ++n) {
+    float v[MR][4];
+#pragma unroll
+    for (int m = 0; m < MR; ++m)
+#pragma unroll
+      for (int i = 0; i < 4; ++i) v[m][i] = acc[m][n][i] + bias[m][i];
+    const uint32_t vo = (__umul24(opx[n], (uint32_t)a.out0_cs) + a.out0_co + cq) * 2;
+    v4u32 pk[MR / 2 > 0 ? MR / 2 : 1];
+    uint32_t off[MR / 2 > 0 ? MR / 2 : 1];
+    epi_col<MR, ACT, RES>(v, rq[n], vo, pv[n], cout0, a.Cout, quad, pk, off, ep.pk1[n], ep.off1[n]);
+#pragma unroll
+    for (int m = 0; m + 1 < MR; m += 2) {
+      ep.pk[m / 2][n] = pk[m / 2];
+      ep.off[m / 2][n] = off[m / 2];
+    }
+  }
+}
+
 template <int MR, int NR>
 __device__ __forceinline__ void epi_pack(const ConvArgs& a, f32x4 (&acc)[MR][NR], int cout0,
                                          const bool (&pv)[NR], const uint32_t (&opx)[NR], int quad,
                                          const f32x4 (&bias)[MR], EpiPend<MR, NR>& ep) {
-  const __amdgpu_buffer_rsrc_t rr =
-      __builtin_amdgcn_make_buffer_rsrc((void*)a.res, 0, 0x7FFFFFFF, kRsrcFlags);
-  const int cq = cout0 + quad * 4;
-  constexpr uint32_t kDrop = 0x80000000u;
-  uint2 rq[MR][NR];
-  if (a.res) {
-#pragma unroll
-    for (int n = 0; n < NR; ++n) {
-      const uint32_t vr = (__umul24(opx[n], (uint32_t)a.res_cs) + a.res_co + cq) * 2;
-#pragma unroll
-      for (int m = 0; m < MR; ++m) {
-        const uint32_t roff = pv[n] && cout0 + m * 16 < a.Cout ? vr + m * 32 : kDrop;
-        rq[m][n] = __builtin_bit_cast(uint2, __builtin_amdgcn_raw_buffer_load_b64(rr, (int)roff, 0, 0));
-      }
-    }
-  }
-  auto value = [&](int m, int n, uint32_t vr, uint32_t& lo, uint32_t& hi) {
-    (void)vr;
-    float v[4];
-#pragma unroll
-    for (int i = 0; i < 4; ++i) v[i] = acc[m][n][i] + bias[m][i];
-    if (a.act) silu4(v);
-    if (a.res) {
-      const uint2 q = rq[m][n];
-      v[0] += bf2f(q.x & 0xFFFF);
-      v[1] += bf2f(q.x >> 16);
-      v[2] += bf2f(q.y & 0xFFFF);
-      v[3] += bf2f(q.y >> 16);
-    }
-    lo = pack_bf16x2(v[0], v[1]);
-    hi = pack_bf16x2(v[2], v[3]);
-  };
-#pragma unroll
-  for (int n = 0; n < NR; ++n) {
-    const uint32_t vo = (__umul24(opx[n], (uint32_t)a.out0_cs) + a.out0_co + cq) * 2;
-    const uint32_t vr = a.res ? (__umul24(opx[n], (uint32_t)a.res_cs) + a.res_co + cq) * 2 : 0u;
-    const uint32_t vo16 = vo + (16 * (quad & 1) + 8 * (quad >> 1) - 4 * quad) * 2;
-#pragma unroll
-    for (int m = 0; m + 1 < MR; m += 2) {
-      uint32_t a0, a1, b0, b1;
-      value(m, n, vr, a0, a1);
-      value(m + 1, n, vr, b0, b1);
-      const auto x0 = __builtin_amdgcn_permlane16_swap(a0, b0, false, false);
-      const auto x1 = __builtin_amdgcn_permlane16_swap(a1, b1, false, false);
-      const bool ok = pv[n] && cout0 + (m + (quad & 1)) * 16 < a.Cout;
-      ep.off[m / 2][n] = ok ? vo16 + m * 32 : kDrop;
-      ep.pk[m / 2][n] = v4u32{x0[0], x1[0], x0[1], x1[1]};
-    }
-    if constexpr (MR & 1) {
-      constexpr int m = MR - 1;
-      uint32_t lo, hi;
-      value(m, n, vr, lo, hi);
-      ep.off1[n] = pv[n] && cout0 + m * 16 < a.Cout ? vo + m * 32 : kDrop;
-      ep.pk1[n] = v2u32{lo, hi};
-    }
+  if (a.act) {
+    if (a.res) epi_pack_t<MR, NR, true, true>(a, acc, cout0, pv, opx, quad, bias, ep);
+    else epi_pack_t<MR, NR, true, false>(a, acc, cout0, pv, opx, quad, bias, ep);
+  } else {
+    if (a.res) epi_pack_t<MR, NR, false, true>(a, acc, cout0, pv, opx, quad, bias, ep);
+    else epi_pack_t<MR, NR, false, false>(a, acc, cout0, pv, opx, quad, bias, ep);
   }
 }
 
@@ -563,6 +606,14 @@
   }
 }
 
+__device__ __forceinline__ ConvArgs kernarg_conv_args() {
+  auto p = __builtin_amdgcn_kernarg_segment_ptr();
+  asm volatile("" : "+s"(p));
+  ConvArgs r;
+  __builtin_memcpy(&r, (const void*)p, sizeof(ConvArgs));
+  return r;
+}
+
 template <int MR, int NR, int K, int S, bool RESW, bool F8, int NW = 4, bool CH = false>
 __global__ __launch_bounds__(64 * NW, NW == 4 ? 2 : 1) void conv_patch_kernel(ConvArgs a, PatchGeo g) {
   extern __shared__ __attribute__((aligned(16))) uint8_t smem[];
@@ -570,7 +621,7 @@
   constexpr int BC = 16 * MR;
   constexpr int W_BYTES = BC * T2 * 64;
   constexpr int MAXP = patch_maxit<NR, S>();
-  static_assert(MAXP <= 32, "tail mask is 32 bits");
+  static_assert(MAXP <= 16, "slot masks, for_live");
   constexpr int WJ = BC * T2 / 16;
   constexpr int MAXW = (WJ + NW - 1) / NW;
   constexpr int EB = F8 ? 1 : 2;
@@ -608,7 +659,7 @@
   const TileWalk walk = tile_walk(ntiles);
   const int nsteps = walk.count() * ngrp;
   const int npp = g.PH * g.PW;
-  const float inv_pw = 1.0f / (float)g.PW;
+  const float inv_pw = 1.0f / (float)g.PW, inv_c = 1.0f / (float)g.C;
 
   constexpr int PB = patch_pixb<S>(), SL = PB / 16;
   int orow[NR], ocol[NR], boff[NR][K];
@@ -616,7 +667,7 @@
 #pragma unroll
   for (int n = 0; n < NR; ++n) {
     const int q = wave * (NR * 16) + n * 16 + col;
-    orow[n] = q / g.C;
+    orow[n] = (int)(((float)q + 0.5f) * inv_c);
     ocol[n] = q - orow[n] * g.C;
     oin[n] = q < g.R * g.C;
     const int pr = oin[n] ? orow[n] * S : 0, pc = oin[n] ? ocol[n] * S : 0;
@@ -673,41 +724,66 @@
     for (int i = tid; i < BC; i += 64 * NW) ch_b_lds[i] = a.ch_b[i];
   }
   uint32_t tailbad = 0;
-  int lgeo[MAXP];
-#pragma unroll
-  for (int it = 0; it < MAXP; ++it) {
-    const int L = 64 * (wave + NW * it) + lane;
-    const int pix = L / SL, q = L - SL * pix;
-    const int py = (int)(((float)pix + 0.5f) * inv_pw);
-    const int sc = pix - py * g.PW;
+  uint32_t deadbad = 0;
+  uint32_t topbad = 0, botbad = 0, leftbad = 0, rightbad = 0;
+  uint32_t lrel[MAXP];
+#pragma unroll
+  for (int it = 0; it < MAXP; ++it) lrel[it] = 0;
+  const int pix_bytes = a.in_cs * EB;
+  const int nlive = wave < g.pinst ? (g.pinst - wave + NW - 1) / NW : 0;
+  {
+    const int iy_last = (g.tiles_y - 1) * g.R * S - pad, ix_last = (g.tiles_x - 1) * g.C * S - pad;
     const int he = (g.PW + 1) >> 1;
-    const int px = S == 1 ? sc : (sc < he ? 2 * sc : 2 * (sc - he) + 1);
-    const int sq = q ^ swzq<F8>(sc);
-    lgeo[it] = (pix < npp ? py : 4095) | (px << 12) | (sq << 24);
-    if ((nch - 1) * CC + sq * (16 / EB) >= Cin) tailbad |= 1u << it;
+    for_live<MAXP>(nlive, [&](auto itc) {
+      constexpr int it = decltype(itc)::value;
+      const int L = 64 * (wave + NW * it) + lane;
+      const int pix = L / SL, q = L - SL * pix;
+      const int py = (int)(((float)pix + 0.5f) * inv_pw);
+      const int sc = pix - py * g.PW;
+      const int px = S == 1 ? sc : (sc < he ? 2 * sc : 2 * (sc - he) + 1);
+      const int sq = q ^ swzq<F8>(sc);
+      lrel[it] = ((uint32_t)py * (uint32_t)a.Win + (uint32_t)px) * (uint32_t)pix_bytes + sq * 16;
+      const uint32_t bit = 1u << it;
+      if (pix >= npp) deadbad |= bit;
+      if (py < pad) topbad |= bit;
+      if (iy_last + py >= a.Hin) botbad |= bit;
+      if (px < pad) leftbad |= bit;
+      if (ix_last + px >= a.Win) rightbad |= bit;
+      if ((nch - 1) * CC + sq * (16 / EB) >= Cin) tailbad |= bit;
+    });
   }
   const bool has_tail = Cin % CC != 0;
   uint32_t voff[MAXP];
+#pragma unroll
+  for (int it = 0; it < MAXP; ++it) voff[it] = kOOB;
   __amdgpu_buffer_rsrc_t img_rsrc;
-  const int pix_bytes = a.in_cs * EB;
-  auto prep_tile = [&](int ti) {
-    const int b = ti / tiles_img;
-    const int r = ti - b * tiles_img;
-    const int ty = r / g.tiles_x, tx = r - (r / g.tiles_x) * g.tiles_x;
-    const int iy0 = ty * g.R * S - pad, ix0 = tx * g.C * S - pad;
-    const uint8_t* base = (const uint8_t*)a.in + ((size_t)b * a.Hin * a.Win * a.in_cs + in_co) * EB;
+  struct TileXY {
+    int b, ty, tx;
+  };
+  const int step_b = walk.step / tiles_img, step_r = walk.step - step_b * tiles_img;
+  const int step_y = step_r / g.tiles_x, step_x = step_r - step_y * g.tiles_x;
+  auto tile_next = [&](TileXY t) {
+    t.tx += step_x;
+    const bool cx = t.tx >= g.tiles_x;
+    t.tx -= cx ? g.tiles_x : 0;
+    t.ty += step_y + (cx ? 1 : 0);
+    const bool cy = t.ty >= g.tiles_y;
+    t.ty -= cy ? g.tiles_y : 0;
+    t.b += step_b + (cy ? 1 : 0);
+    return t;
+  };
+  auto prep_tile = [&](const TileXY& t) {
+    const int iy0 = t.ty * g.R * S - pad, ix0 = t.tx * g.C * S - pad;
+    const uint8_t* base = (const uint8_t*)a.in + ((size_t)t.b * a.Hin * a.Win * a.in_cs + in_co) * EB;
     img_rsrc = __builtin_amdgcn_make_buffer_rsrc((void*)base, 0,
                                                  (a.Hin * a.Win * a.in_cs - in_co) * EB, kRsrcFlags);
-#pragma unroll
-    for (int it = 0; it < MAXP; ++it) {
-      const int gg = lgeo[it];
-      const int iy = iy0 + (gg & 4095), ix = ix0 + ((gg >> 12) & 4095);
-      const bool ok = (unsigned)iy < (unsigned)a.Hin && (unsigned)ix < (unsigned)a.Win;
-      const uint32_t off = __umul24((uint32_t)(__umul24(iy, a.Win) + ix), (uint32_t)pix_bytes) +
-                           ((gg >> 24) & 3) * 16;
-      const uint32_t m = ok ? 0u : 0xFFFFFFFFu;
-      voff[it] = (off & ~m) | (kOOB & m);
-    }
+    const uint32_t org = (uint32_t)(iy0 * a.Win + ix0) * (uint32_t)pix_bytes;
+    const uint32_t bad = deadbad | (t.ty == 0 ? topbad : 0u) | (t.ty == g.tiles_y - 1 ? botbad : 0u) |
+                         (t.tx == 0 ? leftbad : 0u) | (t.tx == g.tiles_x - 1 ? rightbad : 0u);
+    for_live<MAXP>(nlive, [&](auto itc) {
+      constexpr int it = decltype(itc)::value;
+      voff[it] = (bad >> it) & 1 ? kOOB : lrel[it] + org;
+    });
   };
   const __amdgpu_buffer_rsrc_t w_rsrc = __builtin_amdgcn_make_buffer_rsrc(
       (void*)(wts + (size_t)wc0 * Kp * EB), 0, (wcout_pad - wc0) * Kp * EB, kRsrcFlags);
@@ -724,7 +800,7 @@
 #pragma unroll
     for (int it = 0; it < MAXW; ++it) {
       const int j = wave + NW * it;
-      if (j < WJ) dma16(w_rsrc, Wl + j * 1024, wvoff[it], c * 64);
+      if (NW * (it + 1) <= WJ || j < WJ) dma16(w_rsrc, Wl + j * 1024, wvoff[it], c * 64);
     }
   };
   auto stage = [&](int grp, int buf) {
@@ -734,18 +810,16 @@
       uint8_t* P = stages + buf * stage_bytes + gi * chunk_bytes;
       const bool tail = has_tail && c == nch - 1;
       if (tail) {
-#pragma unroll
-        for (int it = 0; it < MAXP; ++it) {
-          const int j = wave + NW * it;
-          if (j < g.pinst)
-            dma16(img_rsrc, P + j * 1024, tail && ((tailbad >> it) & 1) ? kOOB : voff[it], c * 64);
-        }
+        for_live<MAXP>(nlive, [&](auto itc) {
+          constexpr int it = decltype(itc)::value;
+          dma16(img_rsrc, P + (wave + NW * it) * 1024,
+                voff[it] | ((tailbad << (31 - it)) & 0x80000000u), c * 64);
+        });
       } else {
-#pragma unroll
-        for (int it = 0; it < MAXP; ++it) {
-          const int j = wave + NW * it;
-          if (j < g.pinst) dma16(img_rsrc, P + j * 1024, voff[it], c * 64);
-        }
+        for_live<MAXP>(nlive, [&](auto itc) {
+          constexpr int it = decltype(itc)::value;
+          dma16(img_rsrc, P + (wave + NW * it) * 1024, voff[it], c * 64);
+        });
       }
       if constexpr (!RESW) dma_weights(c, P + g.p_bytes);
     }
@@ -882,35 +956,46 @@
 #else
 #define RV_PH(i)
 #endif
-  int ti = walk.t0;
+  TileXY cur, nxt;
+  {
+    const int b = walk.t0 / tiles_img, r = walk.t0 - b * tiles_img;
+    cur = TileXY{b, r / g.tiles_x, r - (r / g.tiles_x) * g.tiles_x};
+    nxt = cur;
+  }
   int grp = 0;
   constexpr bool kDefer = !F8 && !CH && MR * NR <= 10;
   auto chain_tile = [&](const bool (&pv)[NR], const uint32_t (&opx)[NR]) {
     if constexpr (CH) {
       f32x4 bl[MR];
       bias_tile(bl);
-#pragma unroll
-      for (int n = 0; n < NR; ++n) {
-        const int px = n * 16 + col;
-#pragma unroll
-        for (int m = 0; m < MR; m += 2) {
-          uint32_t v0[2], v1[2];
-#pragma unroll
-          for (int h = 0; h < 2; ++h) {
-            float v[4];
-#pragma unroll
-            for (int i = 0; i < 4; ++i) v[i] = acc[m + h][n][i] + bl[m + h][i];
-            if (a.act) silu4(v);
-            v0[h] = pack_bf16x2(v[0], v[1]);
-            v1[h] = pack_bf16x2(v[2], v[3]);
+      auto produce = [&](auto actc) {
+#pragma unroll
+        for (int n = 0; n < NR; ++n) {
+          const int px = n * 16 + col;
+          float v[MR][4];
+#pragma unroll
+          for (int m = 0; m < MR; ++m)
+#pragma unroll
+            for (int i = 0; i < 4; ++i) v[m][i] = acc[m][n][i] + bl[m][i];
+          if constexpr (decltype(actc)::value) silu4_batch<MR>(v);
+#pragma unroll
+          for (int m = 0; m < MR; m += 2) {
+            uint32_t v0[2], v1[2];
+#pragma unroll
+            for (int h = 0; h < 2; ++h) {
+              v0[h] = pack_bf16x2(v[m + h][0], v[m + h][1]);
+              v1[h] = pack_bf16x2(v[m + h][2], v[m + h][3]);
+            }
+            const auto x0 = __builtin_amdgcn_permlane16_swap(v0[0], v0[1], false, false);
+            const auto x1 = __builtin_amdgcn_permlane16_swap(v1[0], v1[1], false, false);
+            const int qq = 2 * (quad & 1) + (quad >> 1);
+            *(v4u32*)(ch_x_lds + ((m / 2) * NR * 16 + px) * 64 + ((qq ^ swzq<false>(px)) << 4)) =
+                v4u32{x0[0], x1[0], x0[1], x1[1]};
           }
-          const auto x0 = __builtin_amdgcn_permlane16_swap(v0[0], v0[1], false, false);
-          const auto x1 = __builtin_amdgcn_permlane16_swap(v1[0], v1[1], false, false);
-          const int qq = 2 * (quad & 1) + (quad >> 1);
-          *(v4u32*)(ch_x_lds + ((m / 2) * NR * 16 + px) * 64 + ((qq ^ swzq<false>(px)) << 4)) =
-              v4u32{x0[0], x1[0], x0[1], x1[1]};
         }
-      }
+      };
+      if (a.act) produce(std::true_type{});
+      else produce(std::false_type{});
       f32x4 acc2[MR][NR];
 #pragma unroll
       for (int m = 0; m < MR; ++m)
@@ -940,16 +1025,11 @@
       f32x4 bl2[MR];
 #pragma unroll
       for (int m = 0; m < MR; ++m) bl2[m] = *(const f32x4*)(ch_b_lds + m * 16 + quad * 4);
-      ConvArgs a2 = a;
-      a2.act = 1;
-      a2.res = nullptr;
-      epilogue_fast<MR, NR>(a2, acc2, 0, pv, opx, quad, bl2);
-    }
-  };
-  auto finish = [&](int tile, EpiPend<MR, NR>& ep) {
-    const int b = tile / tiles_img;
-    const int r = tile - b * tiles_img;
-    const int ty = r / g.tiles_x, tx = r - (r / g.tiles_x) * g.tiles_x;
+      epilogue_fast_t<MR, NR, true, false>(a, acc2, 0, pv, opx, quad, bl2);
+    }
+  };
+  auto finish = [&](const TileXY& t, EpiPend<MR, NR>& ep) {
+    const int b = t.b, ty = t.ty, tx = t.tx;
     bool pv[NR];
     int pb[NR], py[NR], px[NR];
 #pragma unroll
@@ -979,12 +1059,13 @@
     } else {
       f32x4 bl[MR];
       bias_tile(bl);
-      epilogue<MR, NR>(a, acc, cout0, pv, pb, py, px, quad, bl);
+      const ConvArgs ac = kernarg_conv_args();
+      epilogue<MR, NR>(ac, acc, cout0, pv, pb, py, px, quad, bl);
     }
   };
   if constexpr (RESW)
     for (int c = 0; c < nch; ++c) dma_weights(c, smem + c * W_BYTES);
-  prep_tile(ti);
+  prep_tile(cur);
   stage(0, 0);
   __syncthreads();
   RV_PH(0);
@@ -998,15 +1079,18 @@
     }
     const bool last = grp + 1 == ngrp;
     if (s + 1 < nsteps) {
-      if (last) prep_tile(ti + walk.step);
+      if (last) {
+        nxt = tile_next(cur);
+        prep_tile(nxt);
+      }
       stage(last ? 0 : grp + 1, (s + 1) & 1);
     }
     RV_PH(1);
     compute(grp, s & 1);
     RV_PH(2);
     if (last) {
-      finish(ti, ep);
-      ti += walk.step;
+      finish(cur, ep);
+      cur = nxt;
       grp = 0;
       RV_PH(3);
     } else {
@@ -1076,17 +1160,40 @@
   }
   const bool need_geo = a.in_up || !fast;
   const TileWalk walk = tile_walk(ntiles);
+  uint32_t lpix[NR], loff1[NR], loff2[NR];
+#pragma unroll
+  for (int n = 0; n < NR; ++n) {
+    lpix[n] = wave * 16 * NR + n * 16 + col;
+    loff1[n] = lpix[n] * (uint32_t)a.in_cs * 2 + quad * 16;
+    loff2[n] = lpix[n] * (uint32_t)a.in2_cs * 2 + quad * 16;
+  }
+  auto view_bytes = [&](long pixels, int cs, int co) {
+    const long nb = pixels * cs * 2 - (long)co * 2;
+    return (int)(nb < 0 ? 0 : (nb > 0x7FFFFFFF ? 0x7FFFFFFF : nb));
+  };
   struct Geo {
-    const bf16_t* src[NR];
-    const bf16_t* src2[NR];
+    __amdgpu_buffer_rsrc_t r1, r2;
+    uint32_t off1[NR];
     bool pv[NR];
     int pb[NR], py[NR], px[NR];
   };
   auto geo = [&](int t, Geo& G) {
+    const bool live = t < walk.end;
+    const long p0 = (long)t * (64 * NR);
+    const long rem = live && p0 < npix ? npix - p0 : 0;
+    if (a.in_up)
+      G.r1 = __builtin_amdgcn_make_buffer_rsrc(
+          (void*)(a.in + a.in_co), 0,
+          live ? view_bytes((long)a.B * (a.Ho >> 1) * (a.Wo >> 1), a.in_cs, a.in_co) : 0, kRsrcFlags);
+    else
+      G.r1 = __builtin_amdgcn_make_buffer_rsrc((void*)(a.in + a.in_co + (size_t)p0 * a.in_cs), 0,
+                                               view_bytes(rem, a.in_cs, a.in_co), kRsrcFlags);
+    G.r2 = __builtin_amdgcn_make_buffer_rsrc((void*)(a.in2 + a.in2_co + (size_t)p0 * a.in2_cs), 0,
+                                             a.in2 ? view_bytes(rem, a.in2_cs, a.in2_co) : 0, kRsrcFlags);
 #pragma unroll
     for (int n = 0; n < NR; ++n) {
-      const int p = t * 64 * NR + wave * 16 * NR + n * 16 + col;
-      G.pv[n] = t < walk.end && p < npix;
+      const int p = (int)p0 + (int)lpix[n];
+      G.pv[n] = live && p < npix;
       const int pp = G.pv[n] ? p : 0;
       G.pb[n] = G.py[n] = G.px[n] = 0;
       if (need_geo) {
@@ -1095,20 +1202,23 @@
         G.py[n] = r / a.Wo;
         G.px[n] = r - G.py[n] * a.Wo;
       }
-      const size_t ps = a.in_up ? ((size_t)G.pb[n] * (a.Ho >> 1) + (G.py[n] >> 1)) * (a.Wo >> 1) +
-                                      (G.px[n] >> 1)
-                                : (size_t)pp;
-      G.src[n] = a.in + ps * a.in_cs + a.in_co + quad * 8;
-      G.src2[n] = a.in2 + (size_t)pp * a.in2_cs + a.in2_co + quad * 8 - a.split;
+      G.off1[n] = loff1[n];
+      if (a.in_up) {
+        const uint32_t ps = (uint32_t)((G.pb[n] * (a.Ho >> 1) + (G.py[n] >> 1)) * (a.Wo >> 1) + (G.px[n] >> 1));
+        G.off1[n] = G.pv[n] ? ps * (uint32_t)a.in_cs * 2 + quad * 16 : kOOB;
+      }
     }
   };
   auto load = [&](const Geo& G, int c, uint4 (&B)[NR]) {
     const bool kin = c * 32 + quad * 8 < a.Cin;
     const bool second = a.split > 0 && c * 32 >= a.split;
-#pragma unroll
-    for (int n = 0; n < NR; ++n)
-      B[n] = *(const uint4*)((G.pv[n] && kin) ? (const void*)((second ? G.src2[n] : G.src[n]) + c * 32)
-                                              : (const void*)g_zero16);
+    const __amdgpu_buffer_rsrc_t r = second ? G.r2 : G.r1;
+    const int soff = second ? (c * 32 - a.split) * 2 : c * 64;
+#pragma unroll
+    for (int n = 0; n < NR; ++n) {
+      const uint32_t vo = kin ? (second ? loff2[n] : G.off1[n]) : kOOB;
+      B[n] = __builtin_bit_cast(uint4, __builtin_amdgcn_raw_buffer_load_b128(r, (int)vo, soff, 0));
+    }
   };
   auto mma = [&](int c, const uint4 (&B)[NR], f32x4 (&acc)[MR][NR]) {
     const uint8_t* Wl = smem + c * W_BYTES;
@@ -1127,10 +1237,11 @@
     if (fast) {
       uint32_t opx[NR];
 #pragma unroll
-      for (int n = 0; n < NR; ++n) opx[n] = (uint32_t)(t * 64 * NR + wave * 16 * NR + n * 16 + col);
+      for (int n = 0; n < NR; ++n) opx[n] = (uint32_t)(t * 64 * NR) + lpix[n];
       epilogue_fast<MR, NR>(a, acc, cout0, G.pv, opx, quad, bias);
     } else {
-      epilogue<MR, NR>(a, acc, cout0, G.pv, G.pb, G.py, G.px, quad, bias);
+      const ConvArgs ac = kernarg_conv_args();
+      epilogue<MR, NR>(ac, acc, cout0, G.pv, G.pb, G.py, G.px, quad, bias);
     }
   };
   const int P = (nch + 1) & ~1;
@@ -1321,7 +1432,9 @@
                         (a.split == a.Cin || (a.in2 && a.in2_cs % 8 == 0 && a.in2_co % 8 == 0)));
   return a.k == 1 && a.stride == 1 && a.pad == 0 && a.g2_cout0 <= 0 && a.Hin == a.Ho &&
          a.Win == a.Wo && (c.mr <= T || c.mr == 1) && a.in_cs % 8 == 0 && a.in_co % 8 == 0 &&
-         !a.in8 && vcat_ok && direct_smem(a, c.mr) <= 160 * 1024;
+         !a.in8 && vcat_ok && direct_smem(a, c.mr) <= 160 * 1024 &&
+         (!a.in_up || (double)a.B * (a.Ho >> 1) * (a.Wo >> 1) * a.in_cs * 2 < 2147483647.0) &&
+         (double)a.B * a.Ho * a.Wo < 2147483647.0;
 }
 
 
diff --git a/road-vision-system_amd/csrc/conv_common.h b/road-vision-system_amd/csrc/conv_common.h
--- a/road-vision-system_amd/csrc/conv_common.h
+++ b/road-vision-system_amd/csrc/conv_common.h
@@ -34,6 +34,33 @@
   v[2] = b.x;
   v[3] = b.y;
 }
+template <int N>
+__device__ __forceinline__ void silu4_batch(float (*v)[4]) {
+  const float nl2e = __builtin_bit_cast(float, 0xBFB8AA3Bu);
+  f32x2v x[2 * N], t[2 * N];
+#pragma unroll
+  for (int i = 0; i < N; ++i) {
+    x[2 * i] = f32x2v{v[i][0], v[i][1]};
+    x[2 * i + 1] = f32x2v{v[i][2], v[i][3]};
+  }
+#pragma unroll
+  for (int i = 0; i < 2 * N; ++i) t[i] = x[i] * f32x2v{nl2e, nl2e};
+#pragma unroll
+  for (int i = 0; i < 2 * N; ++i) t[i] = f32x2v{__builtin_amdgcn_exp2f(t[i].x), __builtin_amdgcn_exp2f(t[i].y)};
+#pragma unroll
+  for (int i = 0; i < 2 * N; ++i) t[i] = t[i] + 1.0f;
+#pragma unroll
+  for (int i = 0; i < 2 * N; ++i) t[i] = f32x2v{__builtin_amdgcn_rcpf(t[i].x), __builtin_amdgcn_rcpf(t[i].y)};
+#pragma unroll
+  for (int i = 0; i < 2 * N; ++i) x[i] = x[i] * t[i];
+#pragma unroll
+  for (int i = 0; i < N; ++i) {
+    v[i][0] = x[2 * i].x;
+    v[i][1] = x[2 * i].y;
+    v[i][2] = x[2 * i + 1].x;
+    v[i][3] = x[2 * i + 1].y;
+  }
+}
 
 constexpr int kRsrcFlags = 0x00020000;
 constexpr uint32_t kOOB = 0x80000000u;
```
